# adrelino/mv-lm-icp

Hardware: AMD Instinct MI355X
Metric: ICP iterations/sec (NN+Jacobian+LM) (higher is better)
Workload: dtype f64; 1 GPU; cfg4: multiview 32 views x 200k pts, point-to-plane, SophusSE3 (E=62); views=32, pts_per_view=200000, edges=62, parallelism=single GPU, nn=auto

## Files before the change

mv-lm-icp_amd/csrc/api.cpp:

```cpp
#include <algorithm>
#include <cmath>
#include <cstring>
#include <ctime>
#include <chrono>
#include <condition_variable>
#include <exception>
#include <mutex>
#include <new>
#include <thread>

#include "common.h"
#include "comm.h"
#include "nn_tie.h"
#include "../host/se3.h"

namespace mvicp {

static thread_local char g_err[1024] = "";

void set_error(const char* fmt, ...) {
  va_list ap;
  va_start(ap, fmt);
  vsnprintf(g_err, sizeof(g_err), fmt, ap);
  va_end(ap);
}

int abi_exception() noexcept {
  try { throw; }
  catch (const std::bad_alloc&) { set_error("out of host memory"); }
  catch (const std::exception& e) { set_error("internal error: %s", e.what()); }
  catch (...) { set_error("internal error (unknown exception)"); }
  return MVICP_ERR_INTERNAL;
}

double search_bound(const mvicp_ctx* c, double d2_bound) {
  if (!(c->nn_search_factor > 0.0)) return 1.7976931348623157e308;
  const double f = std::max(1.0, c->nn_search_factor);
  const double b = d2_bound * f * f * (1.0 + 1e-9);
  return std::isfinite(b) ? b : 1.7976931348623157e308;
}

int cached_upload(mvicp_ctx* c, const char* key, const void* src, size_t bytes, void** dptr) {
  mvicp_ctx::CachedTable& t = c->tables[key];
  if (t.d && t.bytes.size() == bytes && std::memcmp(t.bytes.data(), src, bytes) == 0) { *dptr = t.d; return MVICP_OK; }
  MV_HIP(hipStreamSynchronize(c->stream));
  if (bytes > t.cap) {
    if (t.d) MV_HIP(hipFree(t.d));
    t.d = nullptr;
    MV_HIP(hipMalloc(&t.d, std::max<size_t>(bytes, 256)));
    t.cap = std::max<size_t>(bytes, 256);
  }
  MV_HIP(hipMemcpy(t.d, src, bytes, hipMemcpyHostToDevice));
  t.bytes.assign((const char*)src, (const char*)src + bytes);
  *dptr = t.d;
  return MVICP_OK;
}

void scratch_reset(mvicp_ctx* c) { c->scratch_used = 0; }

int scratch_upload(mvicp_ctx* c, const void* src, size_t bytes, void** dptr) {
  const size_t aligned = (bytes + 255) & ~(size_t)255;
  if (c->scratch_used + aligned > c->scratch_bytes) {
    if (c->scratch_used != 0) { set_error("scratch overflow (%zu + %zu > %zu)", c->scratch_used, aligned, c->scratch_bytes); return MVICP_ERR_STATE; }
    MV_HIP(hipStreamSynchronize(c->stream));
    if (c->d_scratch) MV_HIP(hipFree(c->d_scratch));
    c->scratch_bytes = std::max<size_t>(aligned * 4, 1 << 20);
    MV_HIP(hipMalloc((void**)&c->d_scratch, c->scratch_bytes));
  }
  void* d = c->d_scratch + c->scratch_used;
  MV_HIP(hipMemcpyAsync(d, src, bytes, hipMemcpyHostToDevice, c->stream));
  MV_HIP(hipStreamSynchronize(c->stream));
  c->scratch_used += aligned;
  *dptr = d;
  return MVICP_OK;
}

ProfScope::ProfScope(mvicp_ctx* ctx, const char* nm, double bytes) : c(ctx), name(nm), on(ctx->profile) {
  if (on && ctx->profile_level >= 2 && ((std::strncmp(nm, "nn_", 3) != 0 && std::strncmp(nm, "linearize", 9) != 0 && std::strcmp(nm, "comm") != 0) ||
                                        std::strcmp(nm, "nn_tie") == 0)) on = false;
  if (!on) return;
  ProfEntry& pe = c->prof[name];
  auto get = [&]() {
    hipEvent_t ev = nullptr;
    if (!pe.pool.empty()) { ev = pe.pool.back(); pe.pool.pop_back(); }
    else if (hipEventCreate(&ev) != hipSuccess) ev = nullptr;
    return ev;
  };
  a = get(); b = get();
  pe.bytes += bytes;
  if (std::strncmp(nm, "nn_", 3) == 0) { pe.survey_bytes += bytes; pe.queries += bytes / 36.0; }
  pe.launches += 1;
  if (a) (void)hipEventRecord(a, c->stream);
}
ProfScope::~ProfScope() {
  if (!on) return;
  if (b) (void)hipEventRecord(b, c->stream);
  if (a && b) c->prof[name].pending.push_back(std::make_pair(a, b));
}
static double now_ms() {
  timespec ts;
  clock_gettime(CLOCK_MONOTONIC, &ts);
  return ts.tv_sec * 1e3 + ts.tv_nsec * 1e-6;
}
HostScope::HostScope(mvicp_ctx* ctx, const char* nm) : c(ctx), name(nm), t0(0.0), on(ctx->profile) { if (on) t0 = now_ms(); }
HostScope::~HostScope() {
  if (!on) return;
  ProfEntry& pe = c->prof[name];
  pe.ms += now_ms() - t0;
  pe.launches += 1;
}
void prof_collect_lazy(mvicp_ctx* c) {
  for (auto& kv : c->prof) if (kv.second.pending.size() > 256) { prof_collect(c); return; }
}
void prof_collect(mvicp_ctx* c) {
  for (auto& kv : c->prof) {
    ProfEntry& pe = kv.second;
    for (auto& pr : pe.pending) {
      float ms = 0.f;
      if (hipEventSynchronize(pr.second) == hipSuccess && hipEventElapsedTime(&ms, pr.first, pr.second) == hipSuccess) pe.ms += ms;
      pe.pool.push_back(pr.first);
      pe.pool.push_back(pr.second);
    }
    pe.pending.clear();
  }
}

namespace {

template <typename T> int dev_alloc(T** p, size_t n) {
  *p = nullptr;
  if (n == 0) n = 1;
  MV_HIP(hipMalloc((void**)p, sizeof(T) * n));
  return MVICP_OK;
}
template <typename T> void dev_free(T*& p) {
  if (p) (void)hipFree(p);
  p = nullptr;
}

void free_graph(mvicp_ctx* c) {
  dev_free(c->d_esrc); dev_free(c->d_edst); dev_free(c->d_cap_off); dev_free(c->d_count);
  dev_free(c->d_ctl); c->d_nsrc = nullptr; c->d_a = nullptr; c->d_xf = nullptr; c->d_rel = nullptr; c->d_rel2 = nullptr; c->d_dirty = nullptr;
  dev_free(c->d_nn_idx); dev_free(c->d_nn_d2); dev_free(c->d_nn_lb); dev_free(c->d_first); dev_free(c->d_second);
  dev_free(c->d_sblock_off); dev_free(c->d_sel_keys1); dev_free(c->d_sel_keys2); c->n_sblocks = 0;
  dev_free(c->d_cd2); dev_free(c->d_qpos); dev_free(c->d_dirty_slots); dev_free(c->d_dslot_off); dev_free(c->d_stream); dev_free(c->d_cblock_off); dev_free(c->d_cblock_cnt); if (c->d_sel_state) (void)hipFree(c->d_sel_state);
  c->d_sel_state = nullptr; dev_free(c->d_sel_hist); dev_free(c->d_median); dev_free(c->d_chunk_edge); dev_free(c->d_chunk_start);
  dev_free(c->d_chunk_first); dev_free(c->d_partials); dev_free(c->d_out);
  if (c->h_pin) (void)hipHostFree(c->h_pin);
  c->h_pin = nullptr; c->h_pin_doubles = 0; c->d_res_host = nullptr; c->d_blocks_host = nullptr; c->lin_out = nullptr;
  c->census_pending = false; c->spec_ready = false; c->spec2_ready = false; c->spec_arm = false; c->d_spec_host = nullptr; c->d_adev_host = nullptr; c->d_res_target = nullptr; c->d_a_check = nullptr;
  dev_free(c->d_xblock_cnt); c->export_valid = false; c->export_in_flight = false; c->export_chunks = 0;
  for (hipEvent_t ev : c->export_events) (void)hipEventDestroy(ev);
  c->export_events.clear();
  if (c->d_export) (void)hipFree(c->d_export);
  if (c->h_export) (void)hipHostFree(c->h_export);
  c->d_export = nullptr; c->h_export = nullptr; c->export_cap = 0;
  c->E = 0; c->total_cap = 0; c->n_cblocks = 0; c->n_chunks = 0; c->have_corr = false;
}

int bind(mvicp_ctx* c) {
  if (!c) { set_error("null context"); return MVICP_ERR_ARG; }
  MV_HIP(hipSetDevice(c->device));
  return MVICP_OK;
}

double sqrt_bound(double t) {
  double x = t * t;
  while (std::sqrt(x) >= t && x > 0.0) x = std::nextafter(x, 0.0);
  while (std::sqrt(x) < t) x = std::nextafter(x, INFINITY);
  return x;
}

void inverse3(const double* m, double* r) {
#define M(i, j) m[(i) + 3 * (j)]
#define COF(i, j) (M(((i) + 1) % 3, ((j) + 1) % 3) * M(((i) + 2) % 3, ((j) + 2) % 3) - M(((i) + 1) % 3, ((j) + 2) % 3) * M(((i) + 2) % 3, ((j) + 1) % 3))
  const double c00 = COF(0, 0), c10 = COF(1, 0), c20 = COF(2, 0);
  const double det = (c00 * M(0, 0) + c10 * M(1, 0)) + c20 * M(2, 0);
  const double invdet = 1.0 / det;
  r[0] = c00 * invdet; r[3] = c10 * invdet; r[6] = c20 * invdet;
  r[1] = COF(0, 1) * invdet; r[4] = COF(1, 1) * invdet; r[7] = COF(2, 1) * invdet;
  r[2] = COF(0, 2) * invdet; r[5] = COF(1, 2) * invdet; r[8] = COF(2, 2) * invdet;
#undef COF
#undef M
}

void fill_query_xf(const double* Ps, const double* Pd, double* x) {
  double Rd[9];
  for (int j = 0; j < 3; ++j)
    for (int i = 0; i < 3; ++i) { x[i + 3 * j] = Ps[i + 4 * j]; Rd[i + 3 * j] = Pd[i + 4 * j]; }
  for (int i = 0; i < 3; ++i) { x[9 + i] = Ps[12 + i]; x[21 + i] = Pd[12 + i]; }
  inverse3(Rd, x + 12);
}

int ensure_pin(mvicp_ctx* c, size_t doubles) {
  if (doubles <= c->h_pin_doubles) return MVICP_OK;
  if (c->h_pin) MV_HIP(hipHostFree(c->h_pin));
  c->h_pin = nullptr;
  MV_HIP(hipHostMalloc((void**)&c->h_pin, sizeof(double) * doubles, hipHostMallocMapped));
  std::memset(c->h_pin, 0, sizeof(double) * doubles);
  c->h_pin_doubles = doubles;
  return MVICP_OK;
}

}

static void fill_rel_into(mvicp_ctx* c, const double* poses, double* h);
void fill_rel(mvicp_ctx* c, const double* poses) {
  fill_rel_into(c, poses, c->h_pin + c->ctl_r2_off);
}
static void fill_rel_into(mvicp_ctx* c, const double* poses, double* h) {
  for (int e = 0; e < c->E; ++e) {
    const double* Ps = poses + 16 * (size_t)c->esrc[e];
    const double* Pd = poses + 16 * (size_t)c->edst[e];
    double* r = h + (size_t)e * kEdgeRel;
    for (int j = 0; j < 3; ++j)
      for (int i = 0; i < 3; ++i) r[i + 3 * j] = Pd[0 + 4 * i] * Ps[0 + 4 * j] + Pd[1 + 4 * i] * Ps[1 + 4 * j] + Pd[2 + 4 * i] * Ps[2 + 4 * j];
    const double dt[3] = {Ps[12] - Pd[12], Ps[13] - Pd[13], Ps[14] - Pd[14]};
    for (int i = 0; i < 3; ++i) r[9 + i] = Pd[0 + 4 * i] * dt[0] + Pd[1 + 4 * i] * dt[1] + Pd[2 + 4 * i] * dt[2];
  }
}
int upload_rel(mvicp_ctx* c, const double* poses) {
  fill_rel(c, poses);
  MV_HIP(hipMemcpyAsync(c->d_rel, c->h_pin + c->ctl_r2_off, sizeof(double) * c->ctl_r2, hipMemcpyHostToDevice, c->stream));
  return MVICP_OK;
}

int stream_wait(mvicp_ctx* c) {
  if (c->spin_wait) {
    const double t0 = now_ms();
    for (;;) {
      const hipError_t q = hipStreamQuery(c->stream);
      if (q == hipSuccess) return MVICP_OK;
      if (q != hipErrorNotReady) { set_error("hipStreamQuery -> %s", hipGetErrorString(q)); return MVICP_ERR_HIP; }
      if (now_ms() - t0 > 2.0) break;
    }
  }
  MV_HIP(hipStreamSynchronize(c->stream));
  return MVICP_OK;
}

void census_resolve(mvicp_ctx* c) {
  if (!c->census_pending) return;
  c->census_pending = false;
  const unsigned long long* st = c->h_census;
  const double nq = c->census_nq;
  ProfEntry& pe = c->prof[c->census_scope];
  if (c->census_kind == 3) {
    const double hits = (double)st[3];
    pe.bytes += 36.0 * hits + 24.0 * (double)st[4] + 24.0 * (double)st[5] + 32.0 * (double)st[1];
    c->nn_candidates += (double)st[0]; c->nn_nodes += (double)st[1] + (double)st[5]; c->nn_far += (double)st[2]; c->nn_queries += nq; c->nn_hits += hits;
    c->nn_fetched += (double)st[4];
    pe.survey_bytes += 24.0 * (double)st[4] + 8.0 * ((double)st[1] + (double)st[5]);
  } else if (c->census_kind == 2) {
    c->nn_fetched += (double)st[0];
    pe.survey_bytes += 24.0 * (double)st[0] + 8.0 * (double)st[1];
    pe.bytes += 28.0 * (double)st[0] + 24.0 * (double)st[1];
    c->nn_candidates += (double)st[2]; c->nn_nodes += (double)st[1]; c->nn_queries += nq;
    for (int k = 0; k < 4; ++k) c->nn_dbg[k] += (double)st[4 + k];
    c->nn_hits += (double)st[3]; pe.bytes += 36.0 * (double)st[3];
  } else {
    const double hits = (double)st[3], searched = nq - hits;
    pe.bytes += 36.0 * hits + (c->census_kind == 1 ? 4.0 : 132.0) * searched + 32.0 * (double)st[0] + 32.0 * (double)st[1];
    c->nn_candidates += (double)st[0]; c->nn_nodes += (double)st[1]; c->nn_far += (double)st[2]; c->nn_queries += nq; c->nn_hits += hits;
    c->nn_fetched += (double)st[0];
    pe.survey_bytes += 24.0 * (double)st[0] + 8.0 * (double)st[1];
  }
}

namespace {
struct BuildSlots {
  std::mutex m; std::condition_variable cv; int free_slots;
  BuildSlots() : free_slots((int)std::max(2u, std::min(32u, std::thread::hardware_concurrency()))) {}
  void acquire() { std::unique_lock<std::mutex> lk(m); cv.wait(lk, [this]() { return free_slots > 0; }); --free_slots; }
  void release() { { std::lock_guard<std::mutex> lk(m); ++free_slots; } cv.notify_one(); }
};
BuildSlots& build_slots() { static BuildSlots s; return s; }
}

static int upload_sorted_normals(FrameDev& f, const double* nrm) {
  const int n = f.n;
  std::vector<double> sn(3 * (size_t)n);
  for (int i = 0; i < n; ++i) std::memcpy(&sn[3 * (size_t)i], nrm + 3 * (size_t)f.grid.h_order[i], 24);
  MV_HIP(hipMalloc((void**)&f.grid.snor, sizeof(double) * 3 * (size_t)std::max(n, 1)));
  MV_HIP(hipMemcpy(f.grid.snor, sn.data(), sizeof(double) * 3 * (size_t)n, hipMemcpyHostToDevice));
  return MVICP_OK;
}

static bool injected_build_failure(mvicp_ctx* c) {
  if (c->fault_inject_build.load() > 0 && c->fault_inject_build.fetch_sub(1) == 1) { set_error("injected structure-build failure (option fault_inject_build)"); return true; }
  return false;
}

static int build_frame_structures(mvicp_ctx* c, FrameDev& f, const double* xyz, const double* nrm) {
  if (injected_build_failure(c)) return MVICP_ERR_INTERNAL;
  const auto t0 = std::chrono::steady_clock::now();
  MV_CHECK(build_grid(c, f, xyz));
  if (nrm) MV_CHECK(upload_sorted_normals(f, nrm));
  f.build_ms[0] = std::chrono::duration<double, std::milli>(std::chrono::steady_clock::now() - t0).count();
  f.build_ms[1] = -1.0;
  return MVICP_OK;
}

static int build_frame_structures_device(mvicp_ctx* c, FrameDev& f, const DevBounds& b, int grid_curve, double grid_target) {
  if (injected_build_failure(c)) return MVICP_ERR_INTERNAL;
  return build_grid_device(c, f, b, grid_curve, grid_target);
}

int finish_builds(mvicp_ctx* c) {
  for (FrameDev& f : c->frames) {
    if (!f.job) continue;
    int s1 = MVICP_ERR_INTERNAL;
    try { s1 = f.job->fut.get(); } catch (...) { f.job->err = "structure build threw"; }
    if (s1 != MVICP_OK) {
      f.build_error = f.job->err.empty() ? std::string("structure build failed") : f.job->err;
      (void)hipSetDevice(c->device);
      free_grid(f.grid); f.has_grid = false;
    }
    f.job.reset();
  }
  for (size_t i = 0; i < c->frames.size(); ++i)
    if (!c->frames[i].build_error.empty()) {
      set_error("frame %d: %s (upload the cloud again with mvicp_set_frame)", (int)i, c->frames[i].build_error.c_str());
      return MVICP_ERR_STATE;
    }
  return MVICP_OK;
}

static void throttle_builds(mvicp_ctx* c) {
  const int limit = std::max(2, (int)std::min(32u, std::thread::hardware_concurrency()));
  for (;;) {
    int pending = 0;
    BuildJob* oldest = nullptr;
    for (FrameDev& f : c->frames)
      if (f.job && f.job->fut.valid() && f.job->fut.wait_for(std::chrono::seconds(0)) != std::future_status::ready) { if (!oldest) oldest = f.job.get(); ++pending; }
    if (pending < limit || !oldest) return;
    oldest->fut.wait();
  }
}

static int check_evaluable(mvicp_ctx* c, int plane) {
  if (!c->have_corr) { set_error("no correspondences: call mvicp_correspond or mvicp_set_correspondences first"); return MVICP_ERR_STATE; }
  if (plane) {
    for (int e = 0; e < c->E; ++e)
      if (c->owned[e] && c->h_count[e] > 0 && c->frames[c->edst[e]].grid.snor == nullptr) {
        set_error("point-to-plane needs normals on frame %d", c->edst[e]);
        return MVICP_ERR_STATE;
      }
  }
  return MVICP_OK;
}

int evaluate_pair(mvicp_ctx* c, const double* poses_a, const double* poses_b, int plane, int robust, double* out_a, double* out_b) {
  MV_CHECK(check_evaluable(c, plane));
  HostScope hs(c, "host.evaluate");
  const size_t n = (size_t)c->E * MVICP_EDGE_BLOCK;
  fill_rel_into(c, poses_b, c->h_pin + c->ctl_rel2_off);
  fill_rel(c, poses_a);
  MV_HIP(hipMemcpyAsync(c->d_rel2, c->h_pin + c->ctl_rel2_off, sizeof(double) * ((size_t)c->E * kEdgeRel + c->ctl_r2), hipMemcpyHostToDevice, c->stream));
  MV_CHECK(launch_linearize_pair(c, plane, robust, c->d_blocks_host, c->d_blocks2_host));
  MV_CHECK(stream_wait(c));
  std::memcpy(out_a, c->h_pin + c->pin_blocks_off, sizeof(double) * n);
  std::memcpy(out_b, c->h_pin + c->pin_blocks2_off, sizeof(double) * n);
  return MVICP_OK;
}

int evaluate_blocks(mvicp_ctx* c, const double* poses, int plane, int robust, double* out) {
  MV_CHECK(check_evaluable(c, plane));
  HostScope hs(c, "host.evaluate");
  const size_t n = (size_t)c->E * MVICP_EDGE_BLOCK;
  if (c->spec_ready) {
    c->spec_ready = false;
    if (plane == c->spec_q_plane && robust == c->spec_q_robust && c->spec_poses.size() == 16 * (size_t)c->n_frames &&
        std::memcmp(poses, c->spec_poses.data(), sizeof(double) * c->spec_poses.size()) == 0) {
      std::memcpy(out, c->h_pin + c->pin_spec_off, sizeof(double) * n);
      if (c->profile) c->prof["spec.hit"].launches += 1;
      return MVICP_OK;
    }
    c->spec2_ready = false;
  }
  if (c->spec2_ready) {
    c->spec2_ready = false;
    if (plane == c->spec2_plane && robust == c->spec2_robust && c->spec2_poses.size() == 16 * (size_t)c->n_frames &&
        std::memcmp(poses, c->spec2_poses.data(), sizeof(double) * c->spec2_poses.size()) == 0) {
      std::memcpy(out, c->h_pin + c->pin_spec2_off, sizeof(double) * n);
      if (c->profile) c->prof["spec2.hit"].launches += 1;
      c->last_cand_poses.assign(poses, poses + 16 * (size_t)c->n_frames); c->last_cand_plane = plane; c->last_cand_robust = robust;
      return MVICP_OK;
    }
  }
  c->last_cand_poses.assign(poses, poses + 16 * (size_t)c->n_frames); c->last_cand_plane = plane; c->last_cand_robust = robust;
  double* h = c->h_pin + c->pin_blocks_off;
  if (c->comm || c->ar_fn) {
    c->lin_out = c->d_out;
    int st_l = upload_rel(c, poses);
    if (st_l == MVICP_OK && c->fault_inject_eval > 0 && --c->fault_inject_eval == 0) { set_error("injected launch failure (option fault_inject_eval)"); st_l = MVICP_ERR_HIP; }
    if (st_l == MVICP_OK) st_l = launch_linearize(c, plane, robust);
    char local_msg[sizeof(g_err)] = "";
    if (st_l != MVICP_OK) std::memcpy(local_msg, g_err, sizeof(local_msg));
    if (hipMemsetAsync(c->d_out + n, st_l == MVICP_OK ? 0 : 0xFF, sizeof(double), c->stream) != hipSuccess) {
      if (st_l != MVICP_OK) return st_l;
      set_error("hipMemsetAsync of the poison slot failed"); return MVICP_ERR_HIP;
    }
    { ProfScope pc(c, "comm", 8.0 * (double)(n + 1)); MV_CHECK(comm_allreduce_sum(c, c->d_out, n + 1)); }
    double* hx = c->h_pin + c->pin_spec_off;
    MV_HIP(hipMemcpyAsync(hx, c->d_out, sizeof(double) * (n + 1), hipMemcpyDeviceToHost, c->stream));
    MV_CHECK(stream_wait(c));
    if (std::isnan(hx[n])) {
      if (st_l != MVICP_OK) { set_error("%s", local_msg); return st_l; }
      set_error("a peer rank failed before the exchange of this evaluation (poisoned exchange buffer)");
      return MVICP_ERR_COMM;
    }
    std::memcpy(out, hx, sizeof(double) * n);
    return MVICP_OK;
  } else {
    MV_CHECK(upload_rel(c, poses));
    c->lin_out = c->d_blocks_host;
    MV_CHECK(launch_linearize(c, plane, robust));
  }
  MV_CHECK(stream_wait(c));
  std::memcpy(out, h, sizeof(double) * n);
  return MVICP_OK;
}

}

using namespace mvicp;

extern "C" {

const char* mvicp_last_error(void) { return g_err; }
const char* mvicp_version(void) { return "mvicp_hip 0.5 (gfx950)"; }

int mvicp_create(int device, mvicp_ctx** out) try {
  if (!out) { set_error("out is null"); return MVICP_ERR_ARG; }
  *out = nullptr;
  int ndev = 0;
  hipError_t e = hipGetDeviceCount(&ndev);
  if (e != hipSuccess || ndev <= 0) {
    set_error("no HIP device available (%s): libmvicp_hip has no CPU fallback", e == hipSuccess ? "device count 0" : hipGetErrorString(e));
    return MVICP_ERR_HIP;
  }
  if (device < 0 || device >= ndev) { set_error("device %d out of range [0,%d)", device, ndev); return MVICP_ERR_ARG; }
  mvicp_ctx* c = new mvicp_ctx();
  c->device = device;
  MV_HIP(hipSetDevice(device));
  MV_HIP(hipStreamCreateWithFlags(&c->stream, hipStreamNonBlocking));
  *out = c;
  return MVICP_OK;
} MVICP_GUARD_ABI

int mvicp_destroy(mvicp_ctx* c) try {
  if (!c) return MVICP_OK;
  (void)hipSetDevice(c->device);
  (void)finish_builds(c);
  (void)hipStreamSynchronize(c->stream);
  comm_destroy(c);
  free_graph(c);
  for (FrameDev& f : c->frames) { dev_free(f.pts); dev_free(f.nor); free_grid(f.grid); free_tie(f); }
  dev_free(c->d_split_idx); dev_free(c->d_split_d2); dev_free(c->d_scratch);
  free_overlap(c);
  for (auto& kv : c->tables) if (kv.second.d) (void)hipFree(kv.second.d);
  if (c->d_census) (void)hipFree(c->d_census);
  if (c->h_census) (void)hipHostFree(c->h_census);
  if (c->d_tie_list) (void)hipFree(c->d_tie_list);
  if (c->d_tie_count) (void)hipFree(c->d_tie_count);
  if (c->h_tie_seen) (void)hipHostFree(c->h_tie_seen);
  if (c->h_far_seen) (void)hipHostFree(c->h_far_seen);
  if (c->d_far_list) (void)hipFree(c->d_far_list);
  if (c->d_far_count) (void)hipFree(c->d_far_count);
  for (auto& kv : c->prof) {
    for (auto& pr : kv.second.pending) { (void)hipEventDestroy(pr.first); (void)hipEventDestroy(pr.second); }
    for (hipEvent_t ev : kv.second.pool) (void)hipEventDestroy(ev);
  }
  (void)hipStreamDestroy(c->stream);
  delete c;
  return MVICP_OK;
} MVICP_GUARD_ABI

int mvicp_set_num_frames(mvicp_ctx* c, int n_frames) try {
  MV_CHECK(bind(c));
  if (n_frames < 0) { set_error("n_frames < 0"); return MVICP_ERR_ARG; }
  (void)finish_builds(c);
  if (c->E) free_graph(c);
  for (FrameDev& f : c->frames) { dev_free(f.pts); dev_free(f.nor); free_grid(f.grid); free_tie(f); }
  c->frames.assign(n_frames, FrameDev());
  c->n_frames = n_frames;
  return MVICP_OK;
} MVICP_GUARD_ABI

int mvicp_set_frame(mvicp_ctx* c, int frame, const double* xyz, const double* nrm, int n) try {
  MV_CHECK(bind(c));
  if (frame < 0 || frame >= c->n_frames) { set_error("frame %d out of range [0,%d)", frame, c->n_frames); return MVICP_ERR_ARG; }
  if (n < 0 || (n > 0 && !xyz)) { set_error("bad cloud (n=%d)", n); return MVICP_ERR_ARG; }
  if (c->E) { set_error("set frames before mvicp_set_graph"); return MVICP_ERR_STATE; }
  FrameDev& f = c->frames[frame];
  if (f.job) { try { (void)f.job->fut.get(); } catch (...) {} f.job.reset(); }
  dev_free(f.pts); dev_free(f.nor); free_grid(f.grid); free_tie(f);
  f.has_grid = false; f.build_error.clear();
  f.n = n;
  MV_CHECK(dev_alloc(&f.pts, 3 * (size_t)n));
  if (n) MV_HIP(hipMemcpy(f.pts, xyz, sizeof(double) * 3 * (size_t)n, hipMemcpyHostToDevice));
  if (nrm) {
    MV_CHECK(dev_alloc(&f.nor, 3 * (size_t)n));
    if (n) MV_HIP(hipMemcpy(f.nor, nrm, sizeof(double) * 3 * (size_t)n, hipMemcpyHostToDevice));
  }
  f.max_norm = 0.0;
  for (int i = 0; i < n; ++i) {
    const double* p = xyz + 3 * (size_t)i;
    if (!std::isfinite(p[0]) || !std::isfinite(p[1]) || !std::isfinite(p[2])) { set_error("non-finite coordinate in cloud"); return MVICP_ERR_ARG; }
    f.max_norm = std::max(f.max_norm, std::sqrt(p[0] * p[0] + p[1] * p[1] + p[2] * p[2]));
  }
  if (n == 0) return MVICP_OK;
  if (!c->async_build) {
    const int st = build_frame_structures(c, f, xyz, nrm);
    if (st != MVICP_OK) { f.build_error = g_err; free_grid(f.grid); f.has_grid = false; }
    return st;
  }
  throttle_builds(c);
  std::shared_ptr<BuildJob> job = std::make_shared<BuildJob>();
  job->xyz.assign(xyz, xyz + 3 * (size_t)n);
  if (nrm) job->nrm.assign(nrm, nrm + 3 * (size_t)n);
  FrameDev* fp = &f;
  BuildJob* jp = job.get();
  job->fut = std::async(std::launch::async, [c, fp, jp]() -> int {
    build_slots().acquire();
    int st = MVICP_ERR_INTERNAL;
    try {
      st = hipSetDevice(c->device) == hipSuccess ? build_frame_structures(c, *fp, jp->xyz.data(), jp->nrm.empty() ? nullptr : jp->nrm.data()) : MVICP_ERR_HIP;
      if (st != MVICP_OK) jp->err = g_err;
    } catch (const std::exception& e) { jp->err = std::string("structure build: ") + e.what(); }
    catch (...) { jp->err = "structure build threw"; }
    std::vector<double>().swap(jp->xyz); std::vector<double>().swap(jp->nrm);
    build_slots().release();
    return st;
  });
  f.job = job;
  return MVICP_OK;
} MVICP_GUARD_ABI

static int check_device_pointer(mvicp_ctx* c, const void* p, const char* what) {
  hipPointerAttribute_t at;
  std::memset(&at, 0, sizeof(at));
  const hipError_t e = hipPointerGetAttributes(&at, p);
  if (e != hipSuccess) {
    (void)hipGetLastError();
    set_error("%s is not a device pointer (%s)", what, hipGetErrorString(e));
    return MVICP_ERR_ARG;
  }
  if (at.type != hipMemoryTypeDevice) { set_error("%s is not device memory (memory type %d)", what, (int)at.type); return MVICP_ERR_ARG; }
  if (at.device != c->device) { set_error("%s lives on device %d, the context on device %d", what, at.device, c->device); return MVICP_ERR_ARG; }
  return MVICP_OK;
}

int mvicp_set_frame_device(mvicp_ctx* c, int frame, const double* d_xyz, const double* d_nrm, int n) try {
  MV_CHECK(bind(c));
  if (frame < 0 || frame >= c->n_frames) { set_error("frame %d out of range [0,%d)", frame, c->n_frames); return MVICP_ERR_ARG; }
  if (n < 0 || (n > 0 && !d_xyz)) { set_error("bad cloud (n=%d)", n); return MVICP_ERR_ARG; }
  if (c->E) { set_error("set frames before mvicp_set_graph"); return MVICP_ERR_STATE; }
  if (n > 0) {
    MV_CHECK(check_device_pointer(c, d_xyz, "xyz"));
    if (d_nrm) MV_CHECK(check_device_pointer(c, d_nrm, "nrm"));
  }
  FrameDev& f = c->frames[frame];
  if (f.job) { try { (void)f.job->fut.get(); } catch (...) {} f.job.reset(); }
  dev_free(f.pts); dev_free(f.nor); free_grid(f.grid); free_tie(f);
  f.has_grid = false; f.build_error.clear();
  f.n = n;
  f.max_norm = 0.0;
  MV_CHECK(dev_alloc(&f.pts, 3 * (size_t)n));
  if (n) MV_HIP(hipMemcpyAsync(f.pts, d_xyz, sizeof(double) * 3 * (size_t)n, hipMemcpyDeviceToDevice, c->stream));
  if (d_nrm) {
    MV_CHECK(dev_alloc(&f.nor, 3 * (size_t)n));
    if (n) MV_HIP(hipMemcpyAsync(f.nor, d_nrm, sizeof(double) * 3 * (size_t)n, hipMemcpyDeviceToDevice, c->stream));
  }
  if (n == 0) { MV_HIP(hipStreamSynchronize(c->stream)); return MVICP_OK; }
  const auto t0 = std::chrono::steady_clock::now();
  DevBounds b;
  MV_CHECK(device_bounds(c->stream, f.pts, n, &b));
  b.wall_ms = std::chrono::duration<double, std::milli>(std::chrono::steady_clock::now() - t0).count();
  if (b.nonfinite) { set_error("non-finite coordinate in cloud"); return MVICP_ERR_ARG; }
  f.max_norm = b.max_norm;
  const int curve = c->grid_curve;
  const double target = c->grid_target;
  if (!c->async_build) {
    const int st = build_frame_structures_device(c, f, b, curve, target);
    if (st != MVICP_OK) { f.build_error = g_err; free_grid(f.grid); f.has_grid = false; }
    return st;
  }
  throttle_builds(c);
  std::shared_ptr<BuildJob> job = std::make_shared<BuildJob>();
  FrameDev* fp = &f;
  BuildJob* jp = job.get();
  job->fut = std::async(std::launch::async, [c, fp, jp, b, curve, target]() -> int {
    build_slots().acquire();
    int st = MVICP_ERR_INTERNAL;
    try {
      st = hipSetDevice(c->device) == hipSuccess ? build_frame_structures_device(c, *fp, b, curve, target) : MVICP_ERR_HIP;
      if (st != MVICP_OK) jp->err = g_err;
    } catch (const std::exception& e) { jp->err = std::string("structure build: ") + e.what(); }
    catch (...) { jp->err = "structure build threw"; }
    build_slots().release();
    return st;
  });
  f.job = job;
  return MVICP_OK;
} MVICP_GUARD_ABI

long long mvicp_get_structure(mvicp_ctx* c, int frame, const char* name, void* out, long long cap_bytes) try {
  MV_CHECK(bind(c));
  if (frame < 0 || frame >= c->n_frames || !name) { set_error("frame %d out of range [0,%d) or no name", frame, c->n_frames); return MVICP_ERR_ARG; }
  MV_CHECK(finish_builds(c));
  const FrameDev& f = c->frames[frame];
  if (!f.has_grid) { set_error("frame %d has no structures (n = %d)", frame, f.n); return MVICP_ERR_STATE; }
  const GridDev& G = f.grid;
  const size_t n = (size_t)f.n;
  const void* dsrc = nullptr; const void* hsrc = nullptr; size_t bytes = 0;
  std::vector<double> sc;
  const int tiles = (f.n + 31) / 32, blocks = (tiles + 63) / 64;
  if (!std::strcmp(name, "spts")) { dsrc = G.spts; bytes = 24 * n; }
  else if (!std::strcmp(name, "sidx")) { dsrc = G.sidx; bytes = 4 * n; }
  else if (!std::strcmp(name, "srec")) { dsrc = G.srec; bytes = sizeof(PointRec) * n; }
  else if (!std::strcmp(name, "crec")) { dsrc = G.crec; bytes = sizeof(PointRec) * n; }
  else if (!std::strcmp(name, "inv")) { dsrc = G.inv; bytes = 4 * n; }
  else if (!std::strcmp(name, "snor")) { dsrc = G.snor; bytes = G.snor ? 24 * n : 0; }
  else if (!std::strcmp(name, "table")) { dsrc = G.table; bytes = 16 * ((size_t)G.table_mask + 1); }
  else if (!std::strcmp(name, "oct")) { dsrc = G.oct; bytes = 32 * (size_t)(8 * G.oct_first_leaf + 1); }
  else if (!std::strcmp(name, "wide")) { dsrc = G.wide; bytes = 4 * (size_t)(G.wide_off[G.wide_levels - 1] + 6ll * G.wide_cnt[G.wide_levels - 1]); }
  else if (!std::strcmp(name, "mf_ops")) { dsrc = G.mf_ops; bytes = (size_t)std::max(tiles, 1) * 64 * 16; }
  else if (!std::strcmp(name, "mf_blk")) { dsrc = G.mf_blk; bytes = (size_t)std::max(blocks, 1) * 48; }
  else if (!std::strcmp(name, "bricks")) { dsrc = G.bricks; bytes = G.bricks ? 16 * (size_t)G.bdims[0] * G.bdims[1] * G.bdims[2] : 0; }
  else if (!std::strcmp(name, "celltab")) { dsrc = G.celltab; bytes = G.celltab ? G.celltab_bytes : 0; }
  else if (!std::strcmp(name, "h_order")) { hsrc = G.h_order.data(); bytes = 4 * G.h_order.size(); }
  else if (!std::strcmp(name, "h_inv")) { hsrc = G.h_inv.data(); bytes = 4 * G.h_inv.size(); }
  else if (!std::strcmp(name, "scalars") || !std::strcmp(name, "build_ms")) {
    if (name[0] == 's') {
      for (int a = 0; a < 3; ++a) sc.push_back(G.dims[a]);
      for (int a = 0; a < 3; ++a) sc.push_back(G.origin[a]);
      sc.push_back(G.cell); sc.push_back(G.inv_cell); sc.push_back(G.n_cells); sc.push_back(G.table_mask); sc.push_back(G.table_shift);
      sc.push_back(G.oct_leaf); sc.push_back((double)G.oct_first_leaf); sc.push_back(G.wide_levels);
      for (int l = 0; l < 6; ++l) sc.push_back(G.wide_cnt[l]);
      for (int l = 0; l < 6; ++l) sc.push_back((double)G.wide_off[l]);
      sc.push_back(G.maxabs); sc.push_back(G.struct_bytes); sc.push_back(f.max_norm);
      for (int a = 0; a < 3; ++a) sc.push_back(G.bdims[a]);
    } else {
      sc.push_back(f.build_ms[0]); sc.push_back(f.build_ms[1]);
    }
    hsrc = sc.data(); bytes = sizeof(double) * sc.size();
  } else { set_error("unknown structure name \"%s\"", name); return MVICP_ERR_ARG; }
  if (!out) return (long long)bytes;
  if (cap_bytes < (long long)bytes) { set_error("%s: %zu bytes do not fit in %lld", name, bytes, cap_bytes); return MVICP_ERR_ARG; }
  if (bytes == 0) return 0;
  if (hsrc) std::memcpy(out, hsrc, bytes);
  else {
    MV_HIP(hipStreamSynchronize(c->stream));
    MV_HIP(hipMemcpy(out, dsrc, bytes, hipMemcpyDeviceToHost));
  }
  return (long long)bytes;
} MVICP_GUARD_ABI

int mvicp_recompute_normals(mvicp_ctx* c, int frame, int k, double* nrm_out, int* knn_out) try {
  MV_CHECK(bind(c));
  if (frame < 0 || frame >= c->n_frames) { set_error("frame %d out of range", frame); return MVICP_ERR_ARG; }
  MV_CHECK(finish_builds(c));
  FrameDev& f = c->frames[frame];
  if (f.n < k) { set_error("frame %d has %d points < k = %d (common.h:333 asserts >= 3)", frame, f.n, k); return MVICP_ERR_STATE; }
  if (!f.nor) MV_CHECK(dev_alloc(&f.nor, 3 * (size_t)f.n));
  if (!f.grid.snor) MV_CHECK(dev_alloc(&f.grid.snor, 3 * (size_t)f.n));
  int* d_knn = nullptr;
  if (knn_out) MV_CHECK(dev_alloc(&d_knn, (size_t)f.n * k));
  int st = launch_normals(c, f, k, d_knn);
  if (st == MVICP_OK) {
    hipError_t e = hipStreamSynchronize(c->stream);
    if (e == hipSuccess && nrm_out) e = hipMemcpy(nrm_out, f.nor, sizeof(double) * 3 * (size_t)f.n, hipMemcpyDeviceToHost);
    if (e == hipSuccess && knn_out) e = hipMemcpy(knn_out, d_knn, sizeof(int) * (size_t)f.n * k, hipMemcpyDeviceToHost);
    if (e != hipSuccess) { set_error("recompute_normals: %s", hipGetErrorString(e)); st = MVICP_ERR_HIP; }
  }
  dev_free(d_knn);
  c->spec_ready = false; c->spec2_ready = false;
  if (st == MVICP_OK && c->E > 0) {
    bool any = false;
    std::vector<int> dirty(c->E, 0);
    for (int e = 0; e < c->E; ++e)
      if (c->owned[e] && c->edst[e] == frame) { c->list_valid[e] = 0; if (c->have_corr && c->h_count[e] > 0) { dirty[e] = 1; any = true; } }
    if (any) {
      MV_HIP(hipMemcpy(c->d_dirty, dirty.data(), sizeof(int) * c->E, hipMemcpyHostToDevice));
      MV_CHECK(launch_gather_stream(c));
      MV_HIP(hipStreamSynchronize(c->stream));
    }
  }
  if (c->profile) prof_collect_lazy(c);
  return st;
} MVICP_GUARD_ABI

int mvicp_set_shard(mvicp_ctx* c, int rank, int world) try {
  MV_CHECK(bind(c));
  if (world < 1 || rank < 0 || rank >= world) { set_error("bad shard %d/%d", rank, world); return MVICP_ERR_ARG; }
  if (c->E) { set_error("call mvicp_set_shard before mvicp_set_graph"); return MVICP_ERR_STATE; }
  c->rank = rank; c->world = world;
  return MVICP_OK;
} MVICP_GUARD_ABI

int mvicp_edge_owner(int n_edges, const int* n_src, int world, int* owner) try {
  if (n_edges < 0 || world < 1 || (n_edges > 0 && (!n_src || !owner))) { set_error("bad arguments"); return MVICP_ERR_ARG; }
  double total = 0, cum = 0;
  for (int e = 0; e < n_edges; ++e) total += n_src[e];
  for (int e = 0; e < n_edges; ++e) {
    const double n = n_src[e];
    int o = total > 0 ? (int)std::floor((cum + 0.5 * n) * world / total) : 0;
    owner[e] = std::min(std::max(o, 0), world - 1);
    cum += n;
  }
  return MVICP_OK;
} MVICP_GUARD_ABI

int mvicp_overlap(mvicp_ctx* c, const double* poses, float thresh, int max_samples, int* samples, int* hits, long long* sumq, int* q_exp) try {
  MV_CHECK(bind(c));
  if (!poses || !samples || !hits) { set_error("poses / samples / hits is null"); return MVICP_ERR_ARG; }
  if (!std::isfinite(thresh) || !(thresh > 0.f)) { set_error("thresh must be finite and > 0"); return MVICP_ERR_ARG; }
  const int K = c->n_frames;
  if (K <= 0) { set_error("no frames: call mvicp_set_num_frames first"); return MVICP_ERR_STATE; }
  for (size_t k = 0; k < 16 * (size_t)K; ++k)
    if (!std::isfinite(poses[k])) { set_error("non-finite pose entry (frame %d)", (int)(k / 16)); return MVICP_ERR_ARG; }
  for (int i = 0; i < K; ++i)
    if (!c->frames[i].pts) { set_error("frame %d was never uploaded", i); return MVICP_ERR_STATE; }
  MV_CHECK(finish_builds(c));
  const double B2 = sqrt_bound((double)thresh);
  int ex = 0;
  (void)std::frexp(B2, &ex);
  const int q = 31 - ex;
  if (q_exp) *q_exp = q;
  std::vector<double> xf(24 * (size_t)K * K, 0.0);
  for (int i = 0; i < K; ++i)
    for (int j = 0; j < K; ++j)
      if (i != j) fill_query_xf(poses + 16 * (size_t)i, poses + 16 * (size_t)j, &xf[24 * ((size_t)i * K + j)]);
  return overlap_census(c, xf.data(), B2, std::ldexp(1.0, q), max_samples, samples, hits, sumq);
} MVICP_GUARD_ABI

int mvicp_graph_from_overlap(int n_frames, const int* samples, const int* hits, const long long* sumq, int knn, double min_fraction,
                             int skip_frame0, int cap, int* src, int* dst, int* n_components) try {
  const int K = n_frames;
  if (K < 0 || knn < 0 || cap < 0 || (K > 0 && (!samples || !hits)) || !(min_fraction == min_fraction)) { set_error("bad arguments"); return MVICP_ERR_ARG; }
  std::vector<int> parent((size_t)K);
  for (int i = 0; i < K; ++i) parent[i] = i;
  auto root = [&](int a) { while (parent[a] != a) { parent[a] = parent[parent[a]]; a = parent[a]; } return a; };
  int n_edges = 0;
  std::vector<int> cand;
  for (int i = 0; i < K; ++i) {
    cand.clear();
    const int* h = hits + (size_t)i * K;
    const long long* sq = sumq ? sumq + (size_t)i * K : nullptr;
    for (int j = 0; j < K; ++j)
      if (j != i && h[j] > 0 && (double)h[j] >= min_fraction * (double)samples[i]) cand.push_back(j);
    std::sort(cand.begin(), cand.end(), [&](int a, int b) {
      if (h[a] != h[b]) return h[a] > h[b];
      if (sq && sq[a] != sq[b]) return sq[a] < sq[b];
      return a < b;
    });
    const int take = std::min<int>(knn, (int)cand.size());
    for (int k = 0; k < take; ++k) {
      parent[root(i)] = root(cand[k]);
      if (i == 0 && skip_frame0) continue;
      if (n_edges >= cap) { set_error("more than cap = %d edges (frame %d of %d, knn = %d)", cap, i, K, knn); return MVICP_ERR_ARG; }
      if (!src || !dst) { set_error("src / dst is null"); return MVICP_ERR_ARG; }
      src[n_edges] = i; dst[n_edges] = cand[k]; ++n_edges;
    }
  }
  if (n_components) {
    int comps = 0;
    for (int i = 0; i < K; ++i) comps += root(i) == i ? 1 : 0;
    *n_components = comps;
  }
  return n_edges;
} MVICP_GUARD_ABI

int mvicp_set_graph(mvicp_ctx* c, int n_edges, const int* src, const int* dst) try {
  MV_CHECK(bind(c));
  if (n_edges < 0 || (n_edges > 0 && (!src || !dst))) { set_error("bad edge list"); return MVICP_ERR_ARG; }
  for (int e = 0; e < n_edges; ++e)
    if (src[e] < 0 || src[e] >= c->n_frames || dst[e] < 0 || dst[e] >= c->n_frames || src[e] == dst[e]) {
      set_error("edge %d (%d->%d) invalid", e, src[e], dst[e]);
      return MVICP_ERR_ARG;
    }
  MV_CHECK(finish_builds(c));
  free_graph(c);
  const int E = n_edges;
  c->E = E;
  c->esrc.assign(src, src + E);
  c->edst.assign(dst, dst + E);
  c->owned.assign(E, 0);
  c->active.assign(E, 0);
  c->h_count.assign(E, 0);
  c->h_weight.assign(E, 0.f);
  {
    std::vector<int> ns(E), owner(E);
    for (int e = 0; e < E; ++e) ns[e] = c->frames[src[e]].n;
    MV_CHECK(mvicp_edge_owner(E, ns.data(), c->world, owner.data()));
    for (int e = 0; e < E; ++e) c->owned[e] = owner[e] == c->rank;
  }
  {
    double total = 0;
    for (int e = 0; e < E; ++e) total += c->frames[src[e]].n;
    c->lin_chunk = total >= 6e6 ? 8192 : total >= 2e6 ? 4096 : total >= 5e5 ? 1024 : 512;
    if (c->lin_chunk_override > 0) c->lin_chunk = c->lin_chunk_override;
  }
  const int kLinChunk = c->lin_chunk;
  c->cap_off.assign(E + 1, 0);
  c->cblock_off.assign(E + 1, 0);
  c->chunk_first.assign(E + 1, 0);
  std::vector<int> chunk_edge, chunk_start;
  for (int e = 0; e < E; ++e) {
    const long long n = c->owned[e] ? c->frames[src[e]].n : 0;
    c->cap_off[e + 1] = c->cap_off[e] + ((n + 63) / 64) * 64;
    c->cblock_off[e + 1] = c->cblock_off[e] + (int)((n + kCompactBlock - 1) / kCompactBlock);
    const int nch = (int)((n + kLinChunk - 1) / kLinChunk);
    c->chunk_first[e + 1] = c->chunk_first[e] + nch;
    for (int k = 0; k < nch; ++k) { chunk_edge.push_back(e); chunk_start.push_back(k * kLinChunk); }
  }
  c->total_cap = c->cap_off[E];
  c->n_cblocks = c->cblock_off[E];
  c->n_chunks = c->chunk_first[E];
  if (c->lin_interleave) {
    std::vector<int> ce, cs;
    for (int e0 = 0; e0 < E;) {
      int e1 = e0 + 1;
      while (e1 < E && src[e1] == src[e0]) ++e1;
      int maxc = 0;
      for (int e = e0; e < e1; ++e) maxc = std::max(maxc, c->chunk_first[e + 1] - c->chunk_first[e]);
      for (int g = 0; g < maxc; g += 8)
        for (int e = e0; e < e1; ++e) {
          const int nch = c->chunk_first[e + 1] - c->chunk_first[e];
          for (int k = g; k < std::min(g + 8, nch); ++k) { ce.push_back(e); cs.push_back(k * kLinChunk); }
        }
      e0 = e1;
    }
    chunk_edge.swap(ce); chunk_start.swap(cs);
  }
  const size_t cap = (size_t)c->total_cap;
  MV_CHECK(dev_alloc(&c->d_esrc, E)); MV_CHECK(dev_alloc(&c->d_edst, E)); MV_CHECK(dev_alloc(&c->d_cap_off, E + 1));
  MV_CHECK(dev_alloc(&c->d_count, E));
  c->ctl_r1 = (size_t)E * kEdgeXf + (size_t)E + 2 * (size_t)E;
  c->ctl_rel2_off = (c->ctl_r1 + 1) & ~(size_t)1;
  c->ctl_r2_off = c->ctl_rel2_off + (size_t)E * kEdgeRel;
  c->ctl_r2 = (size_t)E * (kEdgeRel + 1);
  MV_CHECK(dev_alloc(&c->d_ctl, c->ctl_r2_off + c->ctl_r2));
  MV_HIP(hipMemset(c->d_ctl, 0, sizeof(double) * std::max<size_t>(c->ctl_r2_off + c->ctl_r2, 1)));
  c->d_xf = c->d_ctl; c->d_nsrc = reinterpret_cast<int*>(c->d_ctl + (size_t)E * kEdgeXf); c->d_dirty = c->d_nsrc + E;
  c->d_sel_lohi = c->d_ctl + (size_t)E * (kEdgeXf + 1);
  c->sel_med1.assign(E, -1.0); c->sel_med2.assign(E, -1.0);
  c->d_rel = c->d_ctl + c->ctl_r2_off; c->d_a = c->d_rel + (size_t)E * kEdgeRel; c->d_rel2 = c->d_ctl + c->ctl_rel2_off;
  MV_CHECK(dev_alloc(&c->d_nn_idx, cap)); MV_CHECK(dev_alloc(&c->d_nn_d2, cap)); MV_CHECK(dev_alloc(&c->d_nn_lb, cap));
  c->nn_cache_valid = false; c->prev_q.assign((size_t)E * 12, 0.0); c->nn_cache_edge.assign(E, 0);
  c->auto_prev_dist = 0.0; c->auto_last_method = -1; c->corr_tie_seen = c->corr_far_seen = 1u;
  MV_CHECK(dev_alloc(&c->d_first, cap)); MV_CHECK(dev_alloc(&c->d_second, cap)); MV_CHECK(dev_alloc(&c->d_cd2, cap));
  MV_CHECK(dev_alloc(&c->d_stream, 10 * cap));
  MV_CHECK(dev_alloc(&c->d_qpos, cap));
  MV_HIP(hipMemset(c->d_qpos, 0xff, sizeof(int) * std::max<size_t>(cap, 1)));
  c->list_valid.assign(E, 0); c->explicit_list.assign(E, 0); c->export_valid = false; c->export_off.assign((size_t)E + 1, 0);
  c->qpos_valid.assign(E, 0); c->corr_epoch.assign(E, 0);
  for (int e = 0; e < E; ++e) c->corr_epoch[e] = ++c->epoch_counter;
  c->dslot_off.assign(E + 1, 0);
  for (int e = 0; e < E; ++e) c->dslot_off[e + 1] = c->dslot_off[e] + (int)(((c->owned[e] ? c->frames[src[e]].n : 0) + 255) / 256);
  c->n_dslots = c->dslot_off[E];
  MV_CHECK(dev_alloc(&c->d_dirty_slots, (size_t)c->n_dslots)); MV_CHECK(dev_alloc(&c->d_dslot_off, (size_t)E + 1));
  MV_HIP(hipMemset(c->d_dirty_slots, 0, sizeof(int) * std::max<size_t>((size_t)c->n_dslots, 1)));
  MV_HIP(hipMemcpy(c->d_dslot_off, c->dslot_off.data(), sizeof(int) * (E + 1), hipMemcpyHostToDevice));
  MV_CHECK(dev_alloc(&c->d_cblock_off, E + 1)); MV_CHECK(dev_alloc(&c->d_cblock_cnt, (size_t)c->n_cblocks));
  MV_HIP(hipMalloc(&c->d_sel_state, 16 * 3 * (size_t)std::max(E, 1))); MV_CHECK(dev_alloc(&c->d_sel_hist, (size_t)E * (3 * 2048 + 5)));
  c->sblock_off.assign(E + 1, 0);
  for (int e = 0; e < E; ++e) c->sblock_off[e + 1] = c->sblock_off[e] + (int)(((c->owned[e] ? c->frames[src[e]].n : 0) + kSelBlock - 1) / kSelBlock);
  c->n_sblocks = c->sblock_off[E];
  MV_CHECK(dev_alloc(&c->d_sblock_off, (size_t)E + 1));
  MV_HIP(hipMemcpy(c->d_sblock_off, c->sblock_off.data(), sizeof(int) * (E + 1), hipMemcpyHostToDevice));
  MV_CHECK(dev_alloc(&c->d_sel_keys1, cap)); MV_CHECK(dev_alloc(&c->d_sel_keys2, cap));
  if (cap > c->far_cap) {
    if (c->d_far_list) MV_HIP(hipFree(c->d_far_list));
    c->d_far_list = nullptr; c->far_cap = 0;
    MV_HIP(hipMalloc(&c->d_far_list, sizeof(int) * 2 * cap));
    c->far_cap = cap;
  }
  MV_CHECK(warm_nn_grid(c)); MV_CHECK(warm_nn_tile(c)); MV_CHECK(warm_nn_mfma(c));
  if (c->tie_rule && !(c->tie_lazy && c->world == 1)) {
    std::vector<int> need;
    for (int e = 0; e < E; ++e) if (c->owned[e]) need.push_back(dst[e]);
    MV_CHECK(ensure_tie_trees(c, need));
  }
  MV_CHECK(dev_alloc(&c->d_median, E));
  MV_CHECK(dev_alloc(&c->d_chunk_edge, (size_t)c->n_chunks)); MV_CHECK(dev_alloc(&c->d_chunk_start, (size_t)c->n_chunks));
  MV_CHECK(dev_alloc(&c->d_chunk_first, E + 1));
  MV_CHECK(dev_alloc(&c->d_partials, 2 * (size_t)c->n_chunks * kLinPartial));
  MV_CHECK(dev_alloc(&c->d_out, (size_t)E * (MVICP_EDGE_BLOCK + 3) + 2));
  MV_HIP(hipMemset(c->d_out, 0, sizeof(double) * ((size_t)E * (MVICP_EDGE_BLOCK + 3) + 2)));
  if (E) {
    MV_HIP(hipMemcpy(c->d_esrc, src, sizeof(int) * E, hipMemcpyHostToDevice));
    MV_HIP(hipMemcpy(c->d_edst, dst, sizeof(int) * E, hipMemcpyHostToDevice));
    MV_HIP(hipMemset(c->d_count, 0, sizeof(int) * E));
  }
  MV_HIP(hipMemcpy(c->d_cap_off, c->cap_off.data(), sizeof(long long) * (E + 1), hipMemcpyHostToDevice));
  MV_HIP(hipMemcpy(c->d_cblock_off, c->cblock_off.data(), sizeof(int) * (E + 1), hipMemcpyHostToDevice));
  MV_HIP(hipMemcpy(c->d_chunk_first, c->chunk_first.data(), sizeof(int) * (E + 1), hipMemcpyHostToDevice));
  if (c->n_chunks) {
    MV_HIP(hipMemcpy(c->d_chunk_edge, chunk_edge.data(), sizeof(int) * c->n_chunks, hipMemcpyHostToDevice));
    MV_HIP(hipMemcpy(c->d_chunk_start, chunk_start.data(), sizeof(int) * c->n_chunks, hipMemcpyHostToDevice));
  }
  c->pin_blocks_off = c->ctl_r2_off + c->ctl_r2;
  c->pin_res_off = c->pin_blocks_off + (size_t)E * MVICP_EDGE_BLOCK;
  c->pin_misc_off = c->pin_res_off + 2 * (size_t)E + 2;
  c->pin_spec_off = c->pin_misc_off + 4 * (size_t)E + 64;
  c->pin_adev_off = c->pin_spec_off + (size_t)E * (MVICP_EDGE_BLOCK + 3) + 2;
  if (c->h_pin) { MV_HIP(hipHostFree(c->h_pin)); c->h_pin = nullptr; c->h_pin_doubles = 0; }
  c->pin_spec2_off = (c->pin_adev_off + (size_t)E + 8 + 1) & ~(size_t)1;
  c->pin_rel2_off = c->pin_spec2_off + (size_t)E * MVICP_EDGE_BLOCK + ((size_t)E * MVICP_EDGE_BLOCK & 1);
  c->pin_blocks2_off = (c->pin_rel2_off + (size_t)E * kEdgeRel + 1) & ~(size_t)1;
  MV_CHECK(ensure_pin(c, c->pin_blocks2_off + (size_t)E * MVICP_EDGE_BLOCK + 8));
  {
    void* dp = nullptr;
    MV_HIP(hipHostGetDevicePointer(&dp, c->h_pin, 0));
    c->d_blocks_host = (double*)dp + c->pin_blocks_off;
    c->d_res_host = (double*)dp + c->pin_res_off;
    c->d_spec_host = (double*)dp + c->pin_spec_off;
    c->d_adev_host = (double*)dp + c->pin_adev_off;
    c->d_spec2_host = (double*)dp + c->pin_spec2_off;
    c->d_blocks2_host = (double*)dp + c->pin_blocks2_off;
  }
  c->spec_ready = false; c->spec_arm = false; c->bracket_counters_clean = false;
  c->spec2_ready = false; c->spec2_armed = false; c->last_cand_poses.clear();
  c->prev_xf.assign((size_t)E * 24, 0.0);
  if (!c->h_census) MV_HIP(hipHostMalloc((void**)&c->h_census, 8 * sizeof(unsigned long long), hipHostMallocDefault));
  return MVICP_OK;
} MVICP_GUARD_ABI

static void forget_history(mvicp_ctx* c) {
  const int E = c->E;
  c->nn_cache_valid = false; c->nn_cache_thresh = -1.f;
  c->prev_q.assign((size_t)E * 12, 0.0); c->prev_xf.assign((size_t)E * 24, 0.0);
  c->nn_cache_edge.assign(E, 0);
  c->auto_prev_dist = 0.0; c->auto_last_method = -1; c->last_rms = -1.0; c->prev_grid_kernel = false;
  c->corr_tie_seen = c->corr_far_seen = 1u;
  c->list_valid.assign(E, 0);
  c->export_valid = false;
  c->qpos_valid.assign(E, 0);
  for (int e = 0; e < E; ++e) c->corr_epoch[e] = ++c->epoch_counter;
  c->sel_med1.assign(E, -1.0); c->sel_med2.assign(E, -1.0);
  c->spec_ready = false; c->spec_arm = false; c->spec_flags_valid = false;
  c->spec2_ready = false; c->spec2_armed = false; c->last_cand_poses.clear();
  c->have_corr = false;
  std::fill(c->h_count.begin(), c->h_count.end(), 0); std::fill(c->h_weight.begin(), c->h_weight.end(), 0.f);
}

int mvicp_reset_history(mvicp_ctx* c) try {
  MV_CHECK(bind(c));
  MV_HIP(hipStreamSynchronize(c->stream));
  forget_history(c);
  return MVICP_OK;
} MVICP_GUARD_ABI

static int correspond_once(mvicp_ctx* c, const double* poses, const unsigned char* fixed, float thresh, int nn_method, int* counts, float* weights, bool* tie_unresolved);

int mvicp_correspond(mvicp_ctx* c, const double* poses, const unsigned char* fixed, float thresh, int nn_method, int* counts, float* weights) try {
  MV_CHECK(bind(c));
  bool unresolved = false;
  MV_CHECK(correspond_once(c, poses, fixed, thresh, nn_method, counts, weights, &unresolved));
  if (!unresolved) return MVICP_OK;
  std::vector<int> need;
  for (int e = 0; e < c->E; ++e) if (c->active[e] && !c->frames[c->edst[e]].has_tie) need.push_back(c->edst[e]);
  MV_HIP(hipStreamSynchronize(c->stream));
  MV_CHECK(ensure_tie_trees(c, need));
  forget_history(c);
  unresolved = false;
  MV_CHECK(correspond_once(c, poses, fixed, thresh, nn_method, counts, weights, &unresolved));
  if (unresolved) { set_error("tie fix-up still without a tree after building them"); return MVICP_ERR_INTERNAL; }
  return MVICP_OK;
} MVICP_GUARD_ABI

static int correspond_once(mvicp_ctx* c, const double* poses, const unsigned char* fixed, float thresh, int nn_method, int* counts, float* weights, bool* tie_unresolved) {
  if (!poses) { set_error("poses is null"); return MVICP_ERR_ARG; }
  if (c->E == 0) { set_error("no graph: call mvicp_set_graph first"); return MVICP_ERR_STATE; }
  const int E = c->E;
  HostScope hs_all(c, "host.correspond");
  std::vector<int> nsrc(E, 0);
  std::vector<char> same_edge(E, 0);
  std::vector<char> unchanged(E, 0);
  const bool hist_ok = c->have_corr && (int)c->nn_cache_edge.size() == E && c->nn_cache_thresh == thresh && (int)c->qpos_valid.size() == E;
  std::vector<double> eps_ratio;
  bool same_active_set = (int)c->nn_cache_edge.size() == E;
  double* hx = c->h_pin;
  for (int e = 0; e < E; ++e) {
    c->active[e] = c->owned[e] && !(fixed && fixed[c->esrc[e]]);
    if (same_active_set && (c->active[e] != 0) != (c->nn_cache_edge[e] != 0)) same_active_set = false;
    nsrc[e] = c->active[e] ? c->frames[c->esrc[e]].n : 0;
    const double* Ps = poses + 16 * (size_t)c->esrc[e];
    const double* Pd = poses + 16 * (size_t)c->edst[e];
    double* x = hx + (size_t)e * kEdgeXf;
    fill_query_xf(Ps, Pd, x);
    double Mq[12];
    for (int j = 0; j < 3; ++j)
      for (int i = 0; i < 3; ++i) Mq[i + 3 * j] = x[12 + i] * x[0 + 3 * j] + x[12 + i + 3] * x[1 + 3 * j] + x[12 + i + 6] * x[2 + 3 * j];
    const double dt[3] = {x[9] - x[21], x[10] - x[22], x[11] - x[23]};
    for (int i = 0; i < 3; ++i) Mq[9 + i] = x[12 + i] * dt[0] + x[12 + i + 3] * dt[1] + x[12 + i + 6] * dt[2];
    double* pq = &c->prev_q[(size_t)e * 12];
    double scale = 0.0;
    for (int k = 0; k < 12; ++k) { x[25 + k] = Mq[k] - pq[k]; scale = std::max(scale, std::fabs(Mq[k])); }
    const double rmax = c->frames[c->esrc[e]].max_norm;
    if (c->active[e]) {
      double fro = 0.0;
      for (int k = 0; k < 9; ++k) fro += x[25 + k] * x[25 + k];
      const double eps_e = std::sqrt(fro) * rmax + std::sqrt(x[34] * x[34] + x[35] * x[35] + x[36] * x[36]);
      const double mu_e = c->tile_mu * c->frames[c->edst[e]].grid.cell;
      eps_ratio.push_back(mu_e > 0.0 ? eps_e / mu_e : 1e300);
    }
    const bool cache_on = c->nn_cache_valid && c->nn_cache_enable && c->active[e] && (int)c->nn_cache_edge.size() == E && c->nn_cache_edge[e] &&
                          c->nn_cache_thresh == thresh;
    double* pxf = &c->prev_xf[(size_t)e * 24];
    if (!c->owned[e]) unchanged[e] = 1;
    else if (c->active[e]) unchanged[e] = hist_ok && c->nn_cache_edge[e] && c->qpos_valid[e] && !c->explicit_list[e] && std::memcmp(pxf, x, sizeof(double) * 24) == 0;
    else unchanged[e] = hist_ok && !c->nn_cache_edge[e] && !c->explicit_list[e] && c->h_count[e] == 0;
    const bool same_xf = cache_on && std::memcmp(pxf, x, sizeof(double) * 24) == 0;
    x[24] = cache_on ? (same_xf ? 0.0 : 1e-12 * (scale * (rmax + 1.0) + 1.0)) : -1.0;
    same_edge[e] = same_xf;
    std::memcpy(pxf, x, sizeof(double) * 24);
    for (int k = 37; k < kEdgeXf; ++k) x[k] = 0.0;
    std::memcpy(pq, Mq, sizeof(Mq));
  }
  int* hn = reinterpret_cast<int*>(hx + (size_t)E * kEdgeXf);
  int* hd = hn + E;
  std::memcpy(hn, nsrc.data(), sizeof(int) * E);

  int st_local = MVICP_OK;
  if (c->tie_rule && !(c->tie_lazy && c->world == 1)) {
    std::vector<int> need;
    for (int e = 0; e < E; ++e) if (c->active[e] && !c->frames[c->edst[e]].has_tie) need.push_back(c->edst[e]);
    if (!need.empty()) st_local = ensure_tie_trees(c, need);
  }
  const double bound = sqrt_bound((double)thresh);
  double t_mark = now_ms();
  auto mark = [&](const char* nm) { if (c->profile) { const double t = now_ms(); ProfEntry& pe = c->prof[nm]; pe.ms += t - t_mark; pe.launches += 1; t_mark = t; } };
  mark("host.corr.setup");
  int method = nn_method;
  if (method == MVICP_NN_AUTO) {
    method = MVICP_NN_TILE;
    if (c->have_corr) {
      double dist = 0.0, cell = 0.0;
      int m = 0;
      for (int e = 0; e < E; ++e)
        if (c->h_count[e] > 0) { dist += c->h_weight[e] / 1.5; cell += c->frames[c->edst[e]].grid.cell; ++m; }
      if (m > 0) {
        dist /= m; cell /= m;
        const bool settled = c->auto_prev_dist > 0.0 ? dist > c->auto_settle * c->auto_prev_dist : dist < 0.5 * cell;
        if (c->nn_cell) {
          double pred = dist;
          if (c->last_rms >= 0.0) pred = std::min(pred, std::sqrt(c->last_rms * c->last_rms + 0.09 * cell * cell));
          if (pred < c->auto_switch * cell || c->auto_last_method == MVICP_NN_GRID) method = MVICP_NN_GRID;
        } else if (dist < 1.5 * cell && (settled || c->auto_last_method == MVICP_NN_GRID)) method = MVICP_NN_GRID;
        c->auto_prev_dist = dist;
      }
    }
  }
  if (method == MVICP_NN_GRID || method == MVICP_NN_TILE) {
    for (int e = 0; e < E; ++e)
      if (c->active[e] && (!c->frames[c->edst[e]].has_grid || !c->frames[c->esrc[e]].has_grid)) method = MVICP_NN_BRUTE;
  }
  bool tile_lb = false, handed_over = false;
  if (nn_method == MVICP_NN_AUTO && method == MVICP_NN_GRID && c->auto_last_method == MVICP_NN_TILE && c->tile_bounds >= 1 &&
      c->nn_cache_enable && !c->nn_cell) { method = MVICP_NN_TILE; tile_lb = true; handed_over = true; }
  if (method == MVICP_NN_TILE && c->tile_bounds >= 2 && c->nn_cache_enable) tile_lb = true;
  bool tile_cached = false;
  bool all_same = true;
  {
    for (int e = 0; e < E; ++e) if (c->active[e] && !same_edge[e]) all_same = false;
    if (nn_method == MVICP_NN_AUTO && method == MVICP_NN_GRID && !handed_over && c->tile_cache && c->tile_bounds >= 1 && c->nn_cache_valid &&
        c->nn_cache_enable && !c->nn_cell && !all_same) { method = MVICP_NN_TILE; tile_lb = true; tile_cached = true; handed_over = true; }
    if (method == MVICP_NN_TILE && !tile_cached && c->tile_cache >= 2 && tile_lb && c->nn_cache_valid && c->nn_cache_enable && !all_same) tile_cached = true;
  }
  {
    std::vector<int> dirty(E, 1);
    if ((method == MVICP_NN_TILE || (method == MVICP_NN_GRID && !c->nn_tree_only && !c->nn_skip_far)) && c->list_reuse)
      for (int e = 0; e < E; ++e) if (c->active[e] && c->list_valid[e]) dirty[e] = 0;
    std::memcpy(hd, dirty.data(), sizeof(int) * E);
  }
  bool use_bracket = c->sel_bracket && c->have_corr;
  {
    double* lohi = hx + (size_t)E * (kEdgeXf + 1);
    for (int e = 0; e < E; ++e) {
      lohi[2 * e] = lohi[2 * e + 1] = 0.0;
      if (!c->active[e]) continue;
      const double m1 = c->sel_med1[e], m2 = c->sel_med2[e];
      if (!(m1 > 0.0 && m2 > 0.0 && std::fabs(m1 - m2) <= 0.001 * m1)) { use_bracket = false; continue; }
      lohi[2 * e] = m1 * 0.994; lohi[2 * e + 1] = m1 * 1.006;
    }
  }
  bool nothing_can_change = method == MVICP_NN_GRID && c->list_reuse && !c->nn_tree_only && !c->nn_skip_far && same_active_set && !c->nn_cell;
  for (int e = 0; e < E && nothing_can_change; ++e)
    if (c->active[e] && !(same_edge[e] && hd[e] == 0)) nothing_can_change = false;
  c->skip_dirty_reduce = nothing_can_change;
  c->tie_skip = nothing_can_change && c->corr_tie_seen == 0u;
  c->far_skip = nothing_can_change && c->corr_far_seen == 0u && c->prev_grid_kernel && method == MVICP_NN_GRID;
  const bool tie_launched = c->tie_rule && !c->tie_skip, far_launched = method == MVICP_NN_GRID && !c->far_skip;
  const bool exchange = c->comm != nullptr || c->ar_fn != nullptr;
  c->spec_ready = false; c->spec2_ready = false;
  c->spec_arm = c->spec_enable && c->spec_flags_valid;
  if (c->spec_arm && c->spec_plane)
    for (int e = 0; e < E; ++e) if (!(fixed && fixed[c->esrc[e]]) && c->frames[c->edst[e]].n > 0 && c->frames[c->edst[e]].grid.snor == nullptr) c->spec_arm = false;
  const size_t nb = (size_t)E * MVICP_EDGE_BLOCK, ntail = 3 * (size_t)E + 1;
  c->d_res_target = exchange ? c->d_out + nb : nullptr;
  c->d_a_check = exchange ? c->d_out + nb + 2 * (size_t)E + 1 : c->d_adev_host;
  size_t upload_doubles = c->ctl_r1;
  bool spec2_plan = false;
  if (c->spec_arm) {
    c->spec_poses.resize(16 * (size_t)c->n_frames);
    double xp[7];
    for (int k = 0; k < c->n_frames; ++k) { se3::pose_to_x(c->spec_param, poses + 16 * (size_t)k, xp); se3::x_to_pose(c->spec_param, xp, &c->spec_poses[16 * (size_t)k]); }
    fill_rel(c, c->spec_poses.data());
    c->spec_q_plane = c->spec_plane; c->spec_q_robust = c->spec_robust;
    upload_doubles = c->ctl_r2_off + (size_t)E * kEdgeRel;
    spec2_plan = !exchange && c->spec2_enable && all_same && same_active_set && c->have_corr && c->last_cand_poses.size() == 16 * (size_t)c->n_frames &&
                 c->last_cand_plane == c->spec_q_plane && c->last_cand_robust == c->spec_q_robust;
    if (spec2_plan && c->lin_pair) fill_rel_into(c, c->last_cand_poses.data(), hx + c->ctl_rel2_off);
  }
  if (method != MVICP_NN_BRUTE && method != MVICP_NN_GRID && method != MVICP_NN_TILE) { set_error("unknown nn_method %d", nn_method); return MVICP_ERR_ARG; }
  bool all_unchanged = true;
  for (int e = 0; e < E; ++e) { if (!unchanged[e]) all_unchanged = false; if (c->active[e]) c->qpos_valid[e] = 0; }
  auto local_search = [&]() -> int {
  MV_HIP(hipMemcpyAsync(c->d_ctl, hx, sizeof(double) * upload_doubles, hipMemcpyHostToDevice, c->stream));
  c->far_narrow = nn_method == MVICP_NN_AUTO && method == MVICP_NN_GRID && c->nn_cache_valid && c->nn_cache_enable && all_same;
  if (c->fault_inject > 0 && --c->fault_inject == 0) { set_error("injected launch failure (option fault_inject)"); return MVICP_ERR_HIP; }
  if (method == MVICP_NN_BRUTE) MV_CHECK(launch_nn_brute_edges(c));
  else if (method == MVICP_NN_GRID) MV_CHECK(launch_nn_grid_edges(c, bound));
  else {
    c->cached_on_mfma = false;
    if (tile_cached && c->tile_mfma == 1 && c->cache_mfma_ratio > 0.0 && !eps_ratio.empty()) {
      std::nth_element(eps_ratio.begin(), eps_ratio.begin() + eps_ratio.size() / 2, eps_ratio.end());
      const double med = eps_ratio[eps_ratio.size() / 2];
      if (c->profile) { ProfEntry& pe = c->prof["auto.eps_over_mu"]; pe.ms = med; pe.launches += 1; }
      c->cached_on_mfma = med > c->cache_mfma_ratio;
    }
    MV_CHECK(launch_nn_tile_edges(c, bound, tile_lb, tile_cached, c->list_reuse));
  }
  c->tie_skip = false; c->far_skip = false;
  c->prev_grid_kernel = method == MVICP_NN_GRID;
  c->last_rms = -1.0;
  c->nn_cache_valid = ((method == MVICP_NN_GRID) && !c->nn_tree_only && !c->nn_skip_far) || tile_lb;
  c->nn_cache_thresh = thresh;
  c->auto_last_method = handed_over ? MVICP_NN_GRID : method;
  c->nn_cache_edge.assign(c->active.begin(), c->active.end());
  for (int e = 0; e < E; ++e) { c->list_valid[e] = c->active[e]; if (c->owned[e]) c->qpos_valid[e] = c->active[e]; if (c->active[e]) c->explicit_list[e] = 0; }
  if (!all_unchanged) c->export_valid = false;

  mark("host.corr.nn_launch");
  if (!nothing_can_change) {
    MV_CHECK(launch_compact(c, bound));
    MV_CHECK(launch_gather_stream(c));
  }
  return use_bracket ? launch_select_bracket(c) : launch_select_median(c);
  };
  if (st_local == MVICP_OK) st_local = local_search();
  if (st_local != MVICP_OK && !exchange) { c->spec_flags_valid = false; return st_local; }
  int st_q = MVICP_OK;
  char local_msg[sizeof(g_err)] = "";
  if (exchange) {
    c->lin_out = c->d_out;
    if (st_local == MVICP_OK) {
      if (c->spec_arm) st_local = launch_linearize(c, c->spec_q_plane, c->spec_q_robust);
      else {
        if (hipMemsetAsync(c->d_out, 0, sizeof(double) * nb, c->stream) != hipSuccess ||
            hipMemsetAsync(c->d_out + nb + 2 * (size_t)E + 1, 0, sizeof(double) * (size_t)E, c->stream) != hipSuccess) { set_error("hipMemsetAsync of the exchange buffer failed"); st_local = MVICP_ERR_HIP; }
      }
    }
    if (st_local != MVICP_OK) {
      std::memcpy(local_msg, g_err, sizeof(local_msg));
      if (hipMemsetAsync(c->d_out + nb + 2 * (size_t)E, 0xFF, sizeof(double), c->stream) != hipSuccess) {
        set_error("%s — and the exchange buffer could not be poisoned: the peers of this rank will block in the collective", local_msg);
        c->spec_flags_valid = false; c->spec_arm = false;
        return st_local;
      }
    }
    { ProfScope pc(c, "comm", 8.0 * (double)(nb + ntail)); st_q = comm_allreduce_sum(c, c->d_out, nb + ntail); }
    if (st_q == MVICP_OK && hipMemcpyAsync(c->h_pin + c->pin_spec_off, c->d_out, sizeof(double) * (nb + ntail), hipMemcpyDeviceToHost, c->stream) != hipSuccess) {
      set_error("hipMemcpyAsync of the exchanged buffer failed"); st_q = MVICP_ERR_HIP;
    }
  } else if (c->spec_arm && spec2_plan && c->lin_pair) {
    c->spec2_armed = false;
    st_q = launch_linearize_pair(c, c->spec_q_plane, c->spec_q_robust, c->d_spec_host, c->d_spec2_host);
    if (st_q == MVICP_OK) { c->spec2_armed = true; c->spec2_poses = c->last_cand_poses; c->spec2_plane = c->spec_q_plane; c->spec2_robust = c->spec_q_robust; }
  } else if (c->spec_arm) {
    c->lin_out = c->d_spec_host;
    st_q = launch_linearize(c, c->spec_q_plane, c->spec_q_robust);
    c->spec2_armed = false;
    if (st_q == MVICP_OK && spec2_plan) {
      fill_rel_into(c, c->last_cand_poses.data(), c->h_pin + c->pin_rel2_off);
      if (hipMemcpyAsync(c->d_rel, c->h_pin + c->pin_rel2_off, sizeof(double) * (size_t)E * kEdgeRel, hipMemcpyHostToDevice, c->stream) == hipSuccess) {
        c->lin_out = c->d_spec2_host;
        st_q = launch_linearize(c, c->spec_q_plane, c->spec_q_robust);
        if (st_q == MVICP_OK) { c->spec2_armed = true; c->spec2_poses = c->last_cand_poses; c->spec2_plane = c->spec_q_plane; c->spec2_robust = c->spec_q_robust; }
      }
    }
  }
  mark("host.corr.post_launch");
  if (st_q == MVICP_OK) st_q = stream_wait(c);
  if (st_q != MVICP_OK) { c->spec_flags_valid = false; c->spec_arm = false; return st_q; }
  if (exchange && std::isnan(c->h_pin[c->pin_spec_off + nb + 2 * (size_t)E])) {
    forget_history(c);
    c->census_pending = false;
    if (st_local != MVICP_OK) { set_error("%s", local_msg); return st_local; }
    set_error("a peer rank failed before the exchange of this search (poisoned exchange buffer); nothing was updated, cross-round state dropped on every rank");
    return MVICP_ERR_COMM;
  }
  census_resolve(c);
  if (tie_launched) c->corr_tie_seen = c->h_tie_seen ? *c->h_tie_seen : 1u;
  if (tie_launched && c->h_tie_seen && c->h_tie_seen[1] != 0u) *tie_unresolved = true;
  if (far_launched) c->corr_far_seen = c->h_far_seen ? *c->h_far_seen : 1u;
  else if (method != MVICP_NN_GRID) c->corr_far_seen = 1u;
  mark("host.corr.wait");
  const double* hr = exchange ? c->h_pin + c->pin_spec_off + nb : c->h_pin + c->pin_res_off;
  bool spec_bad = false;
  {
    bool redo = false;
    for (int e = 0; e < E; ++e) if (hr[2 * e + 1] < 0.0) redo = true;
    if (redo) {
      spec_bad = true;
      int st_r = launch_select_median(c);
      if (exchange) {
        int st_x = MVICP_OK;
        if (st_r != MVICP_OK) {
          std::memcpy(local_msg, g_err, sizeof(local_msg));
          if (hipMemsetAsync(c->d_out + nb + 2 * (size_t)E, 0xFF, sizeof(double), c->stream) != hipSuccess) { c->spec_flags_valid = false; c->spec_arm = false; return st_r; }
        }
        { ProfScope pc(c, "comm", 8.0 * (double)ntail); st_x = comm_allreduce_sum(c, c->d_out + nb, ntail); }
        if (st_x == MVICP_OK && hipMemcpyAsync(c->h_pin + c->pin_spec_off + nb, c->d_out + nb, sizeof(double) * ntail, hipMemcpyDeviceToHost, c->stream) != hipSuccess) {
          set_error("hipMemcpyAsync of the exchanged tail failed"); st_x = MVICP_ERR_HIP;
        }
        if (st_x == MVICP_OK) st_x = stream_wait(c);
        if (st_x != MVICP_OK) { c->spec_flags_valid = false; c->spec_arm = false; return st_x; }
        if (std::isnan(hr[2 * (size_t)E])) {
          forget_history(c);
          if (st_r != MVICP_OK) { set_error("%s", local_msg); return st_r; }
          set_error("a peer rank failed before the second exchange of this search (poisoned exchange buffer); cross-round state dropped on every rank");
          return MVICP_ERR_COMM;
        }
      } else {
        if (st_r == MVICP_OK) st_r = stream_wait(c);
        if (st_r != MVICP_OK) { c->spec_flags_valid = false; c->spec_arm = false; return st_r; }
      }
    }
  }
  for (int e = 0; e < E; ++e) {
    if (!(c->owned[e] && c->active[e])) { c->sel_med1[e] = c->sel_med2[e] = -1.0; continue; }
    c->sel_med2[e] = c->sel_med1[e];
    c->sel_med1[e] = hr[2 * e] > 0 ? hr[2 * e + 1] : -1.0;
  }
  std::vector<double> pack(2 * (size_t)E, 0.0);
  for (int e = 0; e < E; ++e)
    if (exchange || (c->owned[e] && c->active[e])) { pack[2 * e] = hr[2 * e]; pack[2 * e + 1] = hr[2 * e] > 0 ? hr[2 * e + 1] : 0.0; }
  if (c->spec_arm) {
    const double* ad = exchange ? hr + 2 * (size_t)E + 1 : c->h_pin + c->pin_adev_off;
    if (hr[2 * (size_t)E] != (double)(exchange ? c->world : 1)) spec_bad = true;
    for (int e = 0; e < E && !spec_bad; ++e)
      if (exchange || (c->owned[e] && c->active[e])) {
        const double a_host = pack[2 * e] > 0 ? (double)(float)(std::sqrt(pack[2 * e + 1]) * 1.5) : 0.0;
        if (ad[e] != a_host) spec_bad = true;
      }
  }
  c->spec_ready = c->spec_arm && !spec_bad;
  c->spec2_ready = c->spec_ready && c->spec2_armed;
  c->spec2_armed = false;
  c->spec_arm = false;
  double* ha = c->h_pin + c->ctl_r2_off + (size_t)E * kEdgeRel;
  for (int e = 0; e < E; ++e) {
    c->h_count[e] = (int)pack[2 * e];
    const double nth = std::sqrt(pack[2 * e + 1]);
    c->h_weight[e] = c->h_count[e] > 0 ? (float)(nth * 1.5) : 0.f;
    ha[e] = (double)c->h_weight[e];
    if (counts) counts[e] = c->h_count[e];
    if (weights) weights[e] = c->h_weight[e];
  }
  for (int e = 0; e < E; ++e) if (!unchanged[e]) c->corr_epoch[e] = ++c->epoch_counter;
  c->have_corr = true;
  mark("host.corr.finish");
  if (c->profile) prof_collect_lazy(c);
  return MVICP_OK;
}

static int ensure_export(mvicp_ctx* c, bool wait = true) {
  if (!c->export_valid) {
    HostScope hs(c, "host.export");
    MV_CHECK(launch_export(c));
    c->export_valid = true;
  }
  if (wait && c->export_in_flight) {
    MV_CHECK(stream_wait(c));
    c->export_in_flight = false;
    if (c->profile) prof_collect_lazy(c);
  }
  return MVICP_OK;
}

int mvicp_map_correspondences(mvicp_ctx* c, const mvicp_corr** triples, const long long** offsets) try {
  MV_CHECK(bind(c));
  if (!triples || !offsets) { set_error("null output"); return MVICP_ERR_ARG; }
  if (!c->have_corr) { set_error("no correspondences yet"); return MVICP_ERR_STATE; }
  MV_CHECK(ensure_export(c));
  *triples = (const mvicp_corr*)c->h_export;
  *offsets = c->export_off.data();
  return MVICP_OK;
} MVICP_GUARD_ABI

int mvicp_map_correspondences_async(mvicp_ctx* c, const mvicp_corr** triples, const long long** offsets) try {
  MV_CHECK(bind(c));
  if (!triples || !offsets) { set_error("null output"); return MVICP_ERR_ARG; }
  if (!c->have_corr) { set_error("no correspondences yet"); return MVICP_ERR_STATE; }
  MV_CHECK(ensure_export(c, false));
  *triples = (const mvicp_corr*)c->h_export;
  *offsets = c->export_off.data();
  return MVICP_OK;
} MVICP_GUARD_ABI

int mvicp_wait_correspondences(mvicp_ctx* c, int edge) try {
  MV_CHECK(bind(c));
  if (edge < 0 || edge >= c->E) { set_error("edge %d out of range", edge); return MVICP_ERR_ARG; }
  if (!c->export_valid) { set_error("no export in flight: call mvicp_map_correspondences_async after the search"); return MVICP_ERR_STATE; }
  if (!c->export_in_flight || c->export_chunks == 0) return MVICP_OK;
  const int k = c->export_edge_chunk[edge];
  MV_HIP(hipEventSynchronize(c->export_events[k]));
  if (k == c->export_chunks - 1) c->export_in_flight = false;
  return MVICP_OK;
} MVICP_GUARD_ABI

int mvicp_correspondence_epochs(mvicp_ctx* c, const unsigned long long** epochs) try {
  MV_CHECK(bind(c));
  if (!epochs) { set_error("null output"); return MVICP_ERR_ARG; }
  if (c->E == 0) { set_error("no graph"); return MVICP_ERR_STATE; }
  *epochs = c->corr_epoch.data();
  return MVICP_OK;
} MVICP_GUARD_ABI

int mvicp_get_correspondences(mvicp_ctx* c, int edge, int cap, int* first, int* second, double* dist) try {
  MV_CHECK(bind(c));
  if (edge < 0 || edge >= c->E) { set_error("edge %d out of range", edge); return MVICP_ERR_ARG; }
  if (!c->have_corr) { set_error("no correspondences yet"); return MVICP_ERR_STATE; }
  if (!c->owned[edge]) { set_error("edge %d is owned by another rank", edge); return MVICP_ERR_STATE; }
  const int n = c->h_count[edge];
  if (cap < n) { set_error("capacity %d < count %d", cap, n); return MVICP_ERR_ARG; }
  if (!c->explicit_list[edge]) {
    if (n == 0) return 0;
    MV_CHECK(ensure_export(c));
    const mvicp_corr* t = (const mvicp_corr*)c->h_export + c->export_off[edge];
    if (c->export_off[edge + 1] - c->export_off[edge] != n) { set_error("export of edge %d holds %lld triples, expected %d", edge, c->export_off[edge + 1] - c->export_off[edge], n); return MVICP_ERR_STATE; }
    for (int i = 0; i < n; ++i) {
      if (first) first[i] = t[i].first;
      if (second) second[i] = t[i].second;
      if (dist) dist[i] = t[i].dist;
    }
    return n;
  }
  const size_t off = (size_t)c->cap_off[edge];
  MV_HIP(hipStreamSynchronize(c->stream));
  std::vector<int> a(n), b(n);
  std::vector<double> d(n);
  if (n) {
    MV_HIP(hipMemcpy(a.data(), c->d_first + off, sizeof(int) * n, hipMemcpyDeviceToHost));
    MV_HIP(hipMemcpy(b.data(), c->d_second + off, sizeof(int) * n, hipMemcpyDeviceToHost));
    MV_HIP(hipMemcpy(d.data(), c->d_cd2 + off, sizeof(double) * n, hipMemcpyDeviceToHost));
  }
  const std::vector<int>& so = c->frames[c->esrc[edge]].grid.h_order;
  const std::vector<int>& dorder = c->frames[c->edst[edge]].grid.h_order;
  std::vector<int> perm(n);
  for (int i = 0; i < n; ++i) { a[i] = so[a[i]]; b[i] = dorder[b[i]]; perm[i] = i; }
  std::stable_sort(perm.begin(), perm.end(), [&](int x, int y) { return a[x] < a[y]; });
  for (int i = 0; i < n; ++i) {
    const int k = perm[i];
    if (first) first[i] = a[k];
    if (second) second[i] = b[k];
    if (dist) dist[i] = std::sqrt(d[k]);
  }
  return n;
} MVICP_GUARD_ABI

int mvicp_set_correspondences(mvicp_ctx* c, int edge, int n, const int* first, const int* second, float weight) try {
  MV_CHECK(bind(c));
  if (edge < 0 || edge >= c->E) { set_error("edge %d out of range", edge); return MVICP_ERR_ARG; }
  if (!c->owned[edge]) { set_error("edge %d is owned by another rank", edge); return MVICP_ERR_STATE; }
  const int ns = c->frames[c->esrc[edge]].n, nd = c->frames[c->edst[edge]].n;
  if (n < 0 || n > ns) { set_error("n=%d exceeds the edge capacity N_src=%d", n, ns); return MVICP_ERR_ARG; }
  for (int i = 0; i < n; ++i)
    if (first[i] < 0 || first[i] >= ns || second[i] < 0 || second[i] >= nd) { set_error("correspondence %d out of range", i); return MVICP_ERR_ARG; }
  const size_t off = (size_t)c->cap_off[edge];
  MV_HIP(hipStreamSynchronize(c->stream));
  if (n) {
    const std::vector<int>& si = c->frames[c->esrc[edge]].grid.h_inv;
    const std::vector<int>& di = c->frames[c->edst[edge]].grid.h_inv;
    std::vector<int> a(n), b(n);
    for (int i = 0; i < n; ++i) { a[i] = si[first[i]]; b[i] = di[second[i]]; }
    MV_HIP(hipMemcpy(c->d_first + off, a.data(), sizeof(int) * n, hipMemcpyHostToDevice));
    MV_HIP(hipMemcpy(c->d_second + off, b.data(), sizeof(int) * n, hipMemcpyHostToDevice));
    MV_HIP(hipMemset(c->d_cd2 + off, 0, sizeof(double) * n));
  }
  c->nn_cache_valid = false;
  c->spec_ready = false; c->spec2_ready = false;
  c->list_valid[edge] = 0; c->explicit_list[edge] = 1; c->export_valid = false;
  c->qpos_valid[edge] = 0; c->corr_epoch[edge] = ++c->epoch_counter;
  c->sel_med1[edge] = c->sel_med2[edge] = -1.0;
  const double a = (double)weight;
  MV_HIP(hipMemcpy(c->d_count + edge, &n, sizeof(int), hipMemcpyHostToDevice));
  {
    const int not_identity = -1;
    MV_HIP(hipMemcpy(c->d_nsrc + edge, &not_identity, sizeof(int), hipMemcpyHostToDevice));
  }
  MV_HIP(hipMemcpy(c->d_a + edge, &a, sizeof(double), hipMemcpyHostToDevice));
  c->h_pin[c->ctl_r2_off + (size_t)c->E * kEdgeRel + edge] = a;
  c->h_count[edge] = n;
  c->h_weight[edge] = weight;
  c->have_corr = true;
  const int one = 1;
  MV_HIP(hipMemcpy(c->d_dirty + edge, &one, sizeof(int), hipMemcpyHostToDevice));
  MV_CHECK(launch_gather_stream(c));
  MV_HIP(hipStreamSynchronize(c->stream));
  return MVICP_OK;
} MVICP_GUARD_ABI

int mvicp_nn_query(mvicp_ctx* c, int frame, const double* queries, int n, int nn_method, int* idx, double* d2) try {
  MV_CHECK(bind(c));
  if (frame < 0 || frame >= c->n_frames) { set_error("frame %d out of range", frame); return MVICP_ERR_ARG; }
  if (n < 0 || (n && (!queries || !idx || !d2))) { set_error("bad query buffers"); return MVICP_ERR_ARG; }
  MV_CHECK(finish_builds(c));
  const FrameDev& f = c->frames[frame];
  if (f.n == 0) { set_error("frame %d is empty (nanoflann throws here: nanoflann.hpp:904)", frame); return MVICP_ERR_STATE; }
  if (n == 0) return MVICP_OK;
  double* dq = nullptr; int* di = nullptr; double* dd = nullptr;
  MV_CHECK(dev_alloc(&dq, 3 * (size_t)n)); MV_CHECK(dev_alloc(&di, (size_t)n)); MV_CHECK(dev_alloc(&dd, (size_t)n));
  MV_HIP(hipMemcpy(dq, queries, sizeof(double) * 3 * (size_t)n, hipMemcpyHostToDevice));
  int method = (nn_method == MVICP_NN_AUTO || nn_method == MVICP_NN_TILE) ? MVICP_NN_GRID : nn_method;
  if (c->tie_rule) MV_CHECK(ensure_tie_trees(c, std::vector<int>(1, frame)));
  c->tie_skip = false;
  if (method == MVICP_NN_GRID && !f.has_grid) method = MVICP_NN_BRUTE;
  int st;
  if (method == MVICP_NN_BRUTE) st = launch_nn_brute_queries(c, f, dq, n, di, dd);
  else if (method == MVICP_NN_GRID) st = launch_nn_grid_queries(c, f, dq, n, di, dd);
  else { set_error("unknown nn_method %d", nn_method); st = MVICP_ERR_ARG; }
  if (st == MVICP_OK) {
    hipError_t e1 = hipStreamSynchronize(c->stream);
    if (e1 == hipSuccess) census_resolve(c);
    hipError_t e2 = hipMemcpy(idx, di, sizeof(int) * n, hipMemcpyDeviceToHost);
    hipError_t e3 = hipMemcpy(d2, dd, sizeof(double) * n, hipMemcpyDeviceToHost);
    if (e1 != hipSuccess || e2 != hipSuccess || e3 != hipSuccess) { set_error("nn_query copy-back failed"); st = MVICP_ERR_HIP; }
  }
  dev_free(dq); dev_free(di); dev_free(dd);
  if (c->profile) prof_collect_lazy(c);
  return st;
} MVICP_GUARD_ABI

int mvicp_linearize(mvicp_ctx* c, const double* poses, int point_to_plane, int robust, double* out) try {
  MV_CHECK(bind(c));
  if (!poses || !out) { set_error("null argument"); return MVICP_ERR_ARG; }
  if (c->E == 0) { set_error("no graph"); return MVICP_ERR_STATE; }
  MV_CHECK(evaluate_blocks(c, poses, point_to_plane, robust, out));
  if (c->profile) prof_collect_lazy(c);
  return MVICP_OK;
} MVICP_GUARD_ABI

int mvicp_linearize_pair(mvicp_ctx* c, const double* poses_a, const double* poses_b, int point_to_plane, int robust, double* out_a, double* out_b) try {
  MV_CHECK(bind(c));
  if (!poses_a || !poses_b || !out_a || !out_b) { set_error("null argument"); return MVICP_ERR_ARG; }
  if (c->E == 0) { set_error("no graph"); return MVICP_ERR_STATE; }
  if (c->comm || c->ar_fn) {
    MV_CHECK(evaluate_blocks(c, poses_a, point_to_plane, robust, out_a));
    MV_CHECK(evaluate_blocks(c, poses_b, point_to_plane, robust, out_b));
  } else {
    MV_CHECK(evaluate_pair(c, poses_a, poses_b, point_to_plane, robust, out_a, out_b));
  }
  if (c->profile) prof_collect_lazy(c);
  return MVICP_OK;
} MVICP_GUARD_ABI

int mvicp_set_option(mvicp_ctx* c, const char* name, double value) try {
  MV_CHECK(bind(c));
  if (!name) { set_error("null option name"); return MVICP_ERR_ARG; }
  if (std::strcmp(name, "async_build") == 0) { c->async_build = value != 0.0; return MVICP_OK; }
  if (std::strcmp(name, "grid_target") == 0 || std::strcmp(name, "grid_curve") == 0) MV_CHECK(finish_builds(c));
  if (std::strcmp(name, "nn_tree_only") == 0) { c->nn_tree_only = value != 0.0; return MVICP_OK; }
  if (std::strcmp(name, "nn_cache") == 0) { c->nn_cache_enable = value != 0.0; c->nn_cache_valid = false; return MVICP_OK; }
  if (std::strcmp(name, "lin_chunk") == 0) { c->lin_chunk_override = (int)value; return MVICP_OK; }
  if (std::strcmp(name, "list_reuse") == 0) { c->list_reuse = value != 0.0; return MVICP_OK; }
  if (std::strcmp(name, "lin_interleave") == 0) { c->lin_interleave = value != 0.0; return MVICP_OK; }
  if (std::strcmp(name, "lin_share_p") == 0) { c->lin_share_p = value != 0.0; return MVICP_OK; }
  if (std::strcmp(name, "lin_pair") == 0) { c->lin_pair = value != 0.0; return MVICP_OK; }
  if (std::strcmp(name, "nn_census") == 0) { c->nn_census = value != 0.0; return MVICP_OK; }
  if (std::strcmp(name, "nn_skip_far") == 0) { c->nn_skip_far = value != 0.0; return MVICP_OK; }
  if (std::strcmp(name, "sel_bracket") == 0) { c->sel_bracket = value != 0.0; return MVICP_OK; }
  if (std::strcmp(name, "prune_rho") == 0) { c->prune_rho = value; return MVICP_OK; }
  if (std::strcmp(name, "grid_curve") == 0) { c->grid_curve = (int)value; return MVICP_OK; }
  if (std::strcmp(name, "auto_settle") == 0) { c->auto_settle = value; return MVICP_OK; }
  if (std::strcmp(name, "auto_switch") == 0) { c->auto_switch = value; return MVICP_OK; }
  if (std::strcmp(name, "nn_cell") == 0) { c->nn_cell = value != 0.0; return MVICP_OK; }
  if (std::strcmp(name, "nn_search_factor") == 0) { if (!(value >= 0.0)) { set_error("nn_search_factor < 0"); return MVICP_ERR_ARG; } c->nn_search_factor = value; c->nn_cache_valid = false; return MVICP_OK; }
  if (std::strcmp(name, "tie_rule") == 0) { c->tie_rule = value != 0.0; return MVICP_OK; }
  if (std::strcmp(name, "tie_lazy") == 0) { c->tie_lazy = value != 0.0; return MVICP_OK; }
  if (std::strcmp(name, "tile_seed") == 0) { c->tile_seed = value != 0.0; return MVICP_OK; }
  if (std::strcmp(name, "tile_bounds") == 0) { c->tile_bounds = (int)value; return MVICP_OK; }
  if (std::strcmp(name, "tile_mu") == 0) { if (!(value > 0.0 && value <= 1.0)) { set_error("tile_mu outside (0, 1]"); return MVICP_ERR_ARG; } c->tile_mu = value; return MVICP_OK; }
  if (std::strcmp(name, "mfma_kacc") == 0) { if (!(value >= 1.0 && value <= 1024.0)) { set_error("mfma_kacc outside [1, 1024]"); return MVICP_ERR_ARG; } c->mfma_kacc = value; return MVICP_OK; }
  if (std::strcmp(name, "mfma_lbt") == 0) { c->mfma_lbt = (int)value; return MVICP_OK; }
  if (std::strcmp(name, "mfma_entry") == 0) { c->mfma_entry = (int)value; return MVICP_OK; }
  if (std::strcmp(name, "mfma_trig") == 0) { c->mfma_trig = (int)value; return MVICP_OK; }
  if (std::strcmp(name, "tile_mfma") == 0) { c->tile_mfma = (int)value; return MVICP_OK; }
  if (std::strcmp(name, "tile_waves") == 0) { c->tile_waves = (int)value; return MVICP_OK; }
  if (std::strcmp(name, "cache_mfma_ratio") == 0) { c->cache_mfma_ratio = value; return MVICP_OK; }
  if (std::strcmp(name, "reject_cache") == 0) { c->reject_cache = value != 0.0; return MVICP_OK; }
  if (std::strcmp(name, "tile_miss") == 0) { if (!(value >= 0.0 && value <= 64.0)) { set_error("tile_miss outside [0, 64]"); return MVICP_ERR_ARG; } c->tile_miss = (int)value; return MVICP_OK; }
  if (std::strcmp(name, "tile_cache") == 0) { c->tile_cache = (int)value; return MVICP_OK; }
  if (std::strcmp(name, "spin_wait") == 0) { c->spin_wait = value != 0.0; return MVICP_OK; }
  if (std::strcmp(name, "fault_inject") == 0) { c->fault_inject = (int)value; return MVICP_OK; }
  if (std::strcmp(name, "fault_inject_build") == 0) { c->fault_inject_build.store((int)value); return MVICP_OK; }
  if (std::strcmp(name, "fault_inject_eval") == 0) { c->fault_inject_eval = (int)value; return MVICP_OK; }
  if (std::strcmp(name, "spec_eval") == 0) { c->spec_enable = value != 0.0; c->spec_ready = false; c->spec2_ready = false; return MVICP_OK; }
  if (std::strcmp(name, "spec2_eval") == 0) { c->spec2_enable = value != 0.0; c->spec2_ready = false; return MVICP_OK; }
  if (std::strcmp(name, "grid_target") == 0) {
    if (!(value >= 0.5 && value <= 64.0)) { set_error("grid_target out of range"); return MVICP_ERR_ARG; }
    c->grid_target = value;
    return MVICP_OK;
  }
  set_error("unknown option '%s'", name);
  return MVICP_ERR_ARG;
} MVICP_GUARD_ABI
int mvicp_nn_census_ex(mvicp_ctx* c, double* out, int cap) try {
  MV_CHECK(bind(c));
  if (!out || cap < 0) { set_error("bad output buffer"); return MVICP_ERR_ARG; }
  const double v[10] = {c->nn_queries, c->nn_candidates, c->nn_nodes, c->nn_far, c->nn_hits, c->nn_fetched, c->nn_dbg[0], c->nn_dbg[1], c->nn_dbg[2], c->nn_dbg[3]};
  const int n = std::min(cap, 10);
  for (int i = 0; i < n; ++i) out[i] = v[i];
  return n;
} MVICP_GUARD_ABI
int mvicp_nn_census(mvicp_ctx* c, double* out5) try {
  const int n = mvicp_nn_census_ex(c, out5, 5);
  return n < 0 ? n : MVICP_OK;
} MVICP_GUARD_ABI

int mvicp_profile_enable(mvicp_ctx* c, int on) try {
  MV_CHECK(bind(c));
  c->profile = on != 0;
  c->profile_level = on;
  return MVICP_OK;
} MVICP_GUARD_ABI
int mvicp_profile_reset(mvicp_ctx* c) try {
  MV_CHECK(bind(c));
  MV_HIP(hipStreamSynchronize(c->stream));
  prof_collect(c);
  for (auto& kv : c->prof) { kv.second.ms = 0; kv.second.launches = 0; kv.second.bytes = 0; kv.second.survey_bytes = 0; kv.second.queries = 0; }
  c->nn_candidates = c->nn_nodes = c->nn_far = c->nn_queries = c->nn_hits = c->nn_fetched = 0;
  for (int k = 0; k < 4; ++k) c->nn_dbg[k] = 0;
  return MVICP_OK;
} MVICP_GUARD_ABI
static void prof_sum(mvicp_ctx* c, const char* kernel, double out[5]) {
  for (int k = 0; k < 5; ++k) out[k] = 0.0;
  const std::string key = kernel ? kernel : "";
  for (const auto& kv : c->prof) {
    if (!(kv.first == key || (key == "nn" && kv.first.compare(0, 3, "nn_") == 0))) continue;
    out[0] += kv.second.ms;
    if (key == "nn" && (kv.first == "nn_far" || kv.first == "nn_tie")) continue;
    out[1] += (double)kv.second.launches; out[2] += kv.second.bytes; out[3] += kv.second.survey_bytes; out[4] += kv.second.queries;
  }
}
int mvicp_profile_get(mvicp_ctx* c, const char* kernel, double* total_ms, long long* launches, double* alg_bytes) try {
  MV_CHECK(bind(c));
  MV_HIP(hipStreamSynchronize(c->stream));
  prof_collect(c);
  double v[5];
  prof_sum(c, kernel, v);
  if (total_ms) *total_ms = v[0];
  if (launches) *launches = (long long)v[1];
  if (alg_bytes) *alg_bytes = v[2];
  return MVICP_OK;
} MVICP_GUARD_ABI
int mvicp_profile_get_ex(mvicp_ctx* c, const char* kernel, double* out, int cap) try {
  MV_CHECK(bind(c));
  if (!out || cap < 0) { set_error("bad output buffer"); return MVICP_ERR_ARG; }
  MV_HIP(hipStreamSynchronize(c->stream));
  prof_collect(c);
  double v[5];
  prof_sum(c, kernel, v);
  const int n = std::min(cap, 5);
  for (int k = 0; k < n; ++k) out[k] = v[k];
  return n;
} MVICP_GUARD_ABI
void* mvicp_stream(mvicp_ctx* c) { return c ? (void*)c->stream : nullptr; }
int mvicp_sync(mvicp_ctx* c) try {
  MV_CHECK(bind(c));
  MV_HIP(hipStreamSynchronize(c->stream));
  return MVICP_OK;
} MVICP_GUARD_ABI

}
```

mv-lm-icp_amd/csrc/common.h:

```cpp
#pragma once
#include <hip/hip_runtime.h>

#include <atomic>
#include <cstdarg>
#include <cstdio>
#include <future>
#include <map>
#include <memory>
#include <string>
#include <vector>

#include "../../include/mvicp.h"
#include "abi_guard.h"

namespace mvicp {

void set_error(const char* fmt, ...);

#define MV_HIP(expr)                                                                          \
  do {                                                                                        \
    hipError_t _e = (expr);                                                                   \
    if (_e != hipSuccess) {                                                                   \
      mvicp::set_error("%s:%d: %s -> %s", __FILE__, __LINE__, #expr, hipGetErrorString(_e));  \
      return MVICP_ERR_HIP;                                                                   \
    }                                                                                         \
  } while (0)

#define MV_CHECK(call)            \
  do {                            \
    int _s = (call);              \
    if (_s != MVICP_OK) return _s; \
  } while (0)

constexpr int kLinPartial = 32;
constexpr int kLinThreads = 256;
constexpr int kCompactBlock = 1024;
constexpr int kSelBlock = 8192;
constexpr int kEdgeXf = 40;
constexpr int kEdgeRel = 12;

struct GridDev {
  int dims[3] = {0, 0, 0};
  double origin[3] = {0, 0, 0};
  double cell = 0.0, inv_cell = 0.0;
  int n_cells = 0;
  double* spts = nullptr;
  int* sidx = nullptr;
  void* srec = nullptr;
  void* crec = nullptr;
  double* snor = nullptr;
  int* inv = nullptr;
  std::vector<int> h_order, h_inv;
  void* table = nullptr;
  unsigned int table_mask = 0; int table_shift = 0;
  float* oct = nullptr;
  int oct_leaf = 0; long long oct_first_leaf = 0;
  float* wide = nullptr;
  double maxabs = 0.0;
  int wide_levels = 0;
  int wide_cnt[6] = {0, 0, 0, 0, 0, 0};
  long long wide_off[6] = {0, 0, 0, 0, 0, 0};
  void* mf_ops = nullptr; void* mf_blk = nullptr;
  double struct_bytes = 0.0;
  void* bricks = nullptr; void* celltab = nullptr; int bdims[3] = {0, 0, 0};
  size_t celltab_bytes = 0;
  int* ov_samp = nullptr; int ov_samp_s = 0;
};

struct PointRec { double x, y, z; long long idx; };

struct BuildJob { std::future<int> fut; std::string err; std::vector<double> xyz, nrm; };

struct DevBounds { double lo[3], hi[3], max_norm, maxabs, wall_ms; int nonfinite, pad; };

struct FrameDev {
  std::shared_ptr<BuildJob> job;
  std::string build_error;
  int n = 0;
  double* pts = nullptr;
  double* nor = nullptr;
  GridDev grid;
  bool has_grid = false;
  double max_norm = 0.0;
  double build_ms[2] = {0.0, -1.0};
  void* tie_nodes = nullptr; int* tie_ord = nullptr; int* tie_slot = nullptr; double tie_box[6] = {0, 0, 0, 0, 0, 0}; bool has_tie = false;
};

struct ProfEntry {
  double ms = 0.0;
  long long launches = 0;
  double bytes = 0.0;
  double survey_bytes = 0.0;
  double queries = 0.0;
  std::vector<std::pair<hipEvent_t, hipEvent_t>> pending;
  std::vector<hipEvent_t> pool;
};

struct RcclApi;

}

struct mvicp_ctx {
  int device = 0;
  hipStream_t stream = nullptr;
  int n_frames = 0;
  std::vector<mvicp::FrameDev> frames;

  int rank = 0, world = 1;
  int E = 0;
  std::vector<int> esrc, edst;
  std::vector<char> owned;
  std::vector<long long> cap_off;
  long long total_cap = 0;
  std::vector<int> h_count;
  std::vector<float> h_weight;
  bool have_corr = false;

  double* d_ctl = nullptr; size_t ctl_r1 = 0, ctl_rel2_off = 0, ctl_r2_off = 0, ctl_r2 = 0;
  int* d_esrc = nullptr; int* d_edst = nullptr;
  long long* d_cap_off = nullptr;
  int* d_nsrc = nullptr;
  int* d_count = nullptr;
  double* d_a = nullptr;
  double* d_xf = nullptr;
  double* d_rel = nullptr;
  double* d_rel2 = nullptr;
  int* d_nn_idx = nullptr; double* d_nn_d2 = nullptr;
  float* d_nn_lb = nullptr;
  bool nn_cache_valid = false; bool nn_cache_enable = true; float nn_cache_thresh = -1.f;
  std::vector<char> nn_cache_edge;
  std::vector<double> prev_q;
  std::vector<double> prev_xf;
  int* d_first = nullptr; int* d_second = nullptr; double* d_cd2 = nullptr;
  int* d_qpos = nullptr;
  int* d_dirty = nullptr;
  int* d_dirty_slots = nullptr; int* d_dslot_off = nullptr; std::vector<int> dslot_off; int n_dslots = 0;
  std::vector<char> list_valid;
  std::vector<char> explicit_list;
  void* d_export = nullptr; void* h_export = nullptr; size_t export_cap = 0;
  int* d_xblock_cnt = nullptr;
  std::vector<long long> export_off;
  bool export_valid = false;
  std::vector<hipEvent_t> export_events; std::vector<int> export_edge_chunk; int export_chunks = 0; bool export_in_flight = false;
  std::vector<char> qpos_valid;
  std::vector<unsigned long long> corr_epoch;
  unsigned long long epoch_counter = 0;
  double* d_stream = nullptr;
  int n_cblocks = 0;
  std::vector<int> cblock_off;
  int* d_cblock_off = nullptr; int* d_cblock_cnt = nullptr;
  void* d_sel_state = nullptr; unsigned int* d_sel_hist = nullptr; double* d_median = nullptr;
  int n_sblocks = 0; std::vector<int> sblock_off; int* d_sblock_off = nullptr;
  double* d_sel_lohi = nullptr;
  std::vector<double> sel_med1, sel_med2;
  bool sel_bracket = true;
  bool bracket_counters_clean = false;
  double* d_sel_keys1 = nullptr; double* d_sel_keys2 = nullptr;
  bool lin_interleave = true;
  bool lin_share_p = true;
  int lin_chunk_override = 0;
  int lin_chunk = 4096;
  int n_chunks = 0;
  std::vector<int> chunk_first;
  int* d_chunk_edge = nullptr; int* d_chunk_start = nullptr; int* d_chunk_first = nullptr;
  double* d_partials = nullptr;
  bool lin_pair = true;
  double* d_out = nullptr;
  double* d_res_target = nullptr;
  double* h_pin = nullptr; size_t h_pin_doubles = 0;
  size_t pin_blocks_off = 0, pin_res_off = 0, pin_misc_off = 0;
  double* d_res_host = nullptr;
  double* d_blocks_host = nullptr;
  double* lin_out = nullptr;
  bool spec_enable = true; bool spec_flags_valid = false; int spec_param = 0, spec_plane = 0, spec_robust = 0;
  int spec_q_plane = 0, spec_q_robust = 0;
  bool spec_arm = false;
  bool spec_ready = false;
  std::vector<double> spec_poses;
  size_t pin_spec_off = 0, pin_adev_off = 0; double* d_spec_host = nullptr; double* d_adev_host = nullptr;
  bool spec2_enable = true, spec2_armed = false, spec2_ready = false; int spec2_plane = 0, spec2_robust = 0;
  std::vector<double> spec2_poses;
  std::vector<double> last_cand_poses;
  int last_cand_plane = -1, last_cand_robust = -1;
  size_t pin_spec2_off = 0, pin_rel2_off = 0; double* d_spec2_host = nullptr;
  size_t pin_blocks2_off = 0; double* d_blocks2_host = nullptr;
  double* d_a_check = nullptr;
  bool spin_wait = false;
  unsigned long long* h_census = nullptr;
  bool census_pending = false; double census_nq = 0; int census_kind = 0; const char* census_scope = "nn_grid";
  int* d_split_idx = nullptr; double* d_split_d2 = nullptr; size_t split_cap = 0;

  char* ov_dev = nullptr; char* ov_pin = nullptr; size_t ov_bytes = 0;

  struct CachedTable { std::vector<char> bytes; void* d = nullptr; size_t cap = 0; };
  std::map<std::string, CachedTable> tables;
  char* d_scratch = nullptr; size_t scratch_bytes = 0, scratch_used = 0;
  std::vector<char> active;

  mvicp::RcclApi* rccl = nullptr;
  void* comm = nullptr;
  mvicp_allreduce_fn ar_fn = nullptr; void* ar_user = nullptr;
  std::vector<double> ar_host;

  bool async_build = true;
  std::atomic<int> fault_inject_build{0};
  int fault_inject = 0, fault_inject_eval = 0;
  bool list_reuse = true;
  bool nn_tree_only = false;
  bool nn_census = false;
  void* d_census = nullptr; size_t census_bytes = 0;
  void* d_far_list = nullptr; size_t far_cap = 0; unsigned int* d_far_count = nullptr;
  int far_parity = 0;
  unsigned int* h_far_seen = nullptr; unsigned int* d_far_seen = nullptr;
  bool prev_grid_kernel = false;
  bool far_skip = false;
  bool far_narrow = false;
  bool skip_dirty_reduce = false;
  bool nn_skip_far = false;
  double nn_search_factor = 4.0;
  bool tie_lazy = true;
  bool tie_rule = true;
  unsigned long long* d_tie_list = nullptr; size_t tie_cap = 0; unsigned int* d_tie_count = nullptr; int tie_parity = 0;
  unsigned int* h_tie_seen = nullptr; unsigned int* d_tie_seen = nullptr;
  unsigned int corr_tie_seen = 1u, corr_far_seen = 1u;
  bool tie_skip = false;
  bool tile_seed = true;
  int tile_bounds = 1;
  int tile_cache = 1;
  double cache_mfma_ratio = 3.0;
  bool cached_on_mfma = false;
  bool reject_cache = true;
  int tile_miss = 8;
  double tile_mu = 0.02;
  int tile_mfma = 1;
  double mfma_kacc = 34.0;
  int mfma_lbt = 1;
  int mfma_entry = 0;
  int mfma_trig = 2;
  int tile_waves = 0;
  double auto_prev_dist = 0.0; int auto_last_method = -1; double auto_settle = 0.5;
  double last_rms = -1.0;
  bool nn_cell = false;
  double auto_switch = 1.0;
  double prune_rho = 0.05;
  int grid_curve = 2;
  double grid_target = 5.0;
  double nn_candidates = 0, nn_nodes = 0, nn_far = 0, nn_queries = 0, nn_hits = 0, nn_fetched = 0;
  double nn_dbg[4] = {0, 0, 0, 0};

  bool profile = false; int profile_level = 0;
  std::map<std::string, mvicp::ProfEntry> prof;
};

namespace mvicp {

int launch_nn_brute_edges(mvicp_ctx* c);
int launch_nn_brute_queries(mvicp_ctx* c, const FrameDev& f, const double* d_q, int n, int* d_idx, double* d_d2);
int launch_nn_grid_edges(mvicp_ctx* c, double d2_bound);
double search_bound(const mvicp_ctx* c, double d2_bound);
int launch_nn_tile_edges(mvicp_ctx* c, double d2_bound, bool with_bounds, bool with_cache, bool with_list);
int launch_nn_mfma_edges(mvicp_ctx* c, double d2_bound, bool with_bounds, bool with_cache, bool with_list);
int build_mfma(FrameDev& f, const double* sorted_pts);
int warm_nn_mfma(mvicp_ctx* c);
int warm_nn_tile(mvicp_ctx* c); int warm_nn_grid(mvicp_ctx* c);
int build_wide(FrameDev& f, const double* sorted_pts);
int launch_nn_grid_queries(mvicp_ctx* c, const FrameDev& f, const double* d_q, int n, int* d_idx, double* d_d2);
int build_grid(mvicp_ctx* c, FrameDev& f, const double* h_xyz);
int device_bounds(hipStream_t stream, const double* d_xyz, int n, DevBounds* out);
int build_grid_device(mvicp_ctx* c, FrameDev& f, const DevBounds& b, int grid_curve, double grid_target);
int finish_builds(mvicp_ctx* c);
void free_grid(GridDev& g);
void free_tie(FrameDev& f);
int overlap_census(mvicp_ctx* c, const double* xf, double B2, double scale, int max_samples, int* samples, int* hits, long long* sumq);
void free_overlap(mvicp_ctx* c);
int launch_compact(mvicp_ctx* c, double d2_bound);
int launch_gather_stream(mvicp_ctx* c);
int launch_select_median(mvicp_ctx* c);
int launch_export(mvicp_ctx* c);
int launch_select_bracket(mvicp_ctx* c);
int launch_linearize(mvicp_ctx* c, int plane, int robust);
int launch_linearize_pair(mvicp_ctx* c, int plane, int robust, double* out_a, double* out_b);
int launch_normals(mvicp_ctx* c, FrameDev& f, int k, int* d_knn);
int stream_wait(mvicp_ctx* c);
void census_resolve(mvicp_ctx* c);

int cached_upload(mvicp_ctx* c, const char* key, const void* src, size_t bytes, void** dptr);
void scratch_reset(mvicp_ctx* c);
int scratch_upload(mvicp_ctx* c, const void* src, size_t bytes, void** dptr);

struct ProfScope {
  mvicp_ctx* c; const char* name; hipEvent_t a = nullptr, b = nullptr; bool on;
  ProfScope(mvicp_ctx* c, const char* name, double bytes);
  ~ProfScope();
};
void prof_collect(mvicp_ctx* c);
void prof_collect_lazy(mvicp_ctx* c);
struct HostScope {
  mvicp_ctx* c; const char* name; double t0; bool on;
  HostScope(mvicp_ctx* c, const char* name);
  ~HostScope();
};

}
```

mv-lm-icp_amd/csrc/corr.hip:

```cpp
#include "common.h"

namespace mvicp {

namespace {

constexpr int NT = 256;
constexpr int IPT = kCompactBlock / NT;

__device__ __forceinline__ int find_edge(const int* __restrict__ off, int E, int b) {
  int lo = 0, hi = E;
  while (hi - lo > 1) {
    const int mid = (lo + hi) >> 1;
    if (off[mid] <= b) lo = mid; else hi = mid;
  }
  return lo;
}

__device__ __forceinline__ int block_exclusive_scan(int v, int* __restrict__ wave_tot, int* total) {
  const int lane = threadIdx.x & 63, wave = threadIdx.x >> 6;
  int inc = v;
#pragma unroll
  for (int d = 1; d < 64; d <<= 1) {
    const int o = __shfl_up(inc, d, 64);
    if (lane >= d) inc += o;
  }
  if (lane == 63) wave_tot[wave] = inc;
  __syncthreads();
  int base = 0, tot = 0;
#pragma unroll
  for (int w = 0; w < NT / 64; ++w) {
    const int t = wave_tot[w];
    if (w < wave) base += t;
    tot += t;
  }
  *total = tot;
  return base + inc - v;
}

__global__ __launch_bounds__(NT) void count_kernel(const int* __restrict__ cblock_off, int E, const int* __restrict__ nsrc,
                                                   const long long* __restrict__ cap_off, const int* __restrict__ nn_idx,
                                                   const double* __restrict__ nn_d2, double bound, int* __restrict__ cblock_cnt,
                                                   const int* __restrict__ dirty) {
  __shared__ int wave_tot[NT / 64];
  const int b = blockIdx.x;
  const int e = find_edge(cblock_off, E, b);
  if (dirty[e] == 0) return;
  const int lb = b - cblock_off[e];
  const int n = nsrc[e];
  const long long base = cap_off[e];
  int cnt = 0;
#pragma unroll
  for (int i = 0; i < IPT; ++i) {
    const int k = lb * kCompactBlock + threadIdx.x * IPT + i;
    if (k < n) cnt += (nn_idx[base + k] >= 0 && nn_d2[base + k] < bound) ? 1 : 0;
  }
  int total;
  block_exclusive_scan(cnt, wave_tot, &total);
  if (threadIdx.x == 0) cblock_cnt[b] = total;
}

__global__ __launch_bounds__(NT) void scan_kernel(const int* __restrict__ cblock_off, int* __restrict__ cblock_cnt, int* __restrict__ count,
                                                  const int* __restrict__ dirty) {
  __shared__ int wave_tot[NT / 64];
  __shared__ int carry_s;
  const int e = blockIdx.x;
  if (dirty[e] == 0) return;
  const int b0 = cblock_off[e], b1 = cblock_off[e + 1];
  if (threadIdx.x == 0) carry_s = 0;
  __syncthreads();
  for (int s = b0; s < b1; s += NT) {
    const int b = s + threadIdx.x;
    const int v = (b < b1) ? cblock_cnt[b] : 0;
    int total;
    const int ex = block_exclusive_scan(v, wave_tot, &total);
    const int carry = carry_s;
    if (b < b1) cblock_cnt[b] = carry + ex;
    __syncthreads();
    if (threadIdx.x == 0) carry_s = carry + total;
    __syncthreads();
  }
  if (threadIdx.x == 0) count[e] = carry_s;
}

__global__ __launch_bounds__(NT) void scatter_kernel(const int* __restrict__ cblock_off, int E, const int* __restrict__ nsrc,
                                                     const long long* __restrict__ cap_off, const int* __restrict__ nn_idx,
                                                     const double* __restrict__ nn_d2, double bound, const int* __restrict__ cblock_cnt,
                                                     int* __restrict__ first, int* __restrict__ second, double* __restrict__ cd2,
                                                     int* __restrict__ qpos, const int* __restrict__ dirty) {
  __shared__ int wave_tot[NT / 64];
  const int b = blockIdx.x;
  const int e = find_edge(cblock_off, E, b);
  if (dirty[e] == 0) return;
  const int lb = b - cblock_off[e];
  const int n = nsrc[e];
  const long long base = cap_off[e];
  int idx[IPT];
  double d2[IPT];
  bool ok[IPT];
  int cnt = 0;
#pragma unroll
  for (int i = 0; i < IPT; ++i) {
    const int k = lb * kCompactBlock + threadIdx.x * IPT + i;
    ok[i] = false;
    if (k < n) {
      idx[i] = nn_idx[base + k];
      d2[i] = nn_d2[base + k];
      ok[i] = idx[i] >= 0 && d2[i] < bound;
    }
    cnt += ok[i] ? 1 : 0;
  }
  int total;
  int pos = cblock_cnt[b] + block_exclusive_scan(cnt, wave_tot, &total);
#pragma unroll
  for (int i = 0; i < IPT; ++i) {
    const int k = lb * kCompactBlock + threadIdx.x * IPT + i;
    if (k < n) qpos[base + k] = ok[i] ? pos : -1;
    if (!ok[i]) continue;
    first[base + pos] = k;
    second[base + pos] = idx[i];
    cd2[base + pos] = d2[i];
    ++pos;
  }
}

__global__ __launch_bounds__(NT) void gather_kernel(const int* __restrict__ cblock_off, int E, const int* __restrict__ count,
                                                    const long long* __restrict__ cap_off, long long total_cap, const int* __restrict__ first,
                                                    const int* __restrict__ second, const PointRec* const* __restrict__ src_rec,
                                                    const PointRec* const* __restrict__ dst_rec, const double* const* __restrict__ dst_nor,
                                                    double* __restrict__ stream, const int* __restrict__ dirty) {
  const int b = blockIdx.x;
  const int e = find_edge(cblock_off, E, b);
  if (dirty[e] == 0) return;
  const int lb = b - cblock_off[e];
  const int cnt = count[e];
  if (lb * kCompactBlock >= cnt) return;
  const long long base = cap_off[e];
  const PointRec* __restrict__ sp = src_rec[e];
  const PointRec* __restrict__ dp = dst_rec[e];
  const double* __restrict__ dn = dst_nor[e];
  for (int i = 0; i < IPT; ++i) {
    const int pos = lb * kCompactBlock + i * NT + threadIdx.x;
    if (pos >= cnt) break;
    const size_t f = (size_t)first[base + pos], s = (size_t)second[base + pos];
    const size_t o = (size_t)(base + pos);
    const double2* pa = reinterpret_cast<const double2*>(sp + f);
    const double2 a0 = pa[0], a1 = pa[1];
    const double2* pb = reinterpret_cast<const double2*>(dp + s);
    const double2 b0 = pb[0], b1 = pb[1];
    __builtin_nontemporal_store(a0.x, &stream[0 * total_cap + o]);
    __builtin_nontemporal_store(a0.y, &stream[1 * total_cap + o]);
    __builtin_nontemporal_store(a1.x, &stream[2 * total_cap + o]);
    __builtin_nontemporal_store(b0.x, &stream[7 * total_cap + o]);
    __builtin_nontemporal_store(b0.y, &stream[8 * total_cap + o]);
    __builtin_nontemporal_store(b1.x, &stream[9 * total_cap + o]);
    if (dn != nullptr) {
      const double n0 = dn[3 * s], n1 = dn[3 * s + 1], n2 = dn[3 * s + 2];
      __builtin_nontemporal_store(n0, &stream[3 * total_cap + o]);
      __builtin_nontemporal_store(n1, &stream[4 * total_cap + o]);
      __builtin_nontemporal_store(n2, &stream[5 * total_cap + o]);
      __builtin_nontemporal_store(n0 * b0.x + n1 * b0.y + n2 * b1.x, &stream[6 * total_cap + o]);
    }
  }
}

constexpr int kSelBins = 2048;
struct SelState { unsigned long long prefix; int k; int pad; };

template <int PER, typename F>
__device__ __forceinline__ void pick_bin(F get, unsigned int k, int* __restrict__ wave_tot, int* __restrict__ sh_pick, int& bin, unsigned int& below) {
  unsigned int h[PER];
  int mine = 0;
#pragma unroll
  for (int i = 0; i < PER; ++i) { h[i] = get(threadIdx.x * PER + i); mine += (int)h[i]; }
  int total;
  const int ex = block_exclusive_scan(mine, wave_tot, &total);
  if (threadIdx.x == 0) { sh_pick[0] = NT * PER - 1; sh_pick[1] = total; }
  __syncthreads();
  if ((unsigned int)ex <= k && k < (unsigned int)(ex + mine)) {
    unsigned int cum = (unsigned int)ex;
#pragma unroll
    for (int i = 0; i < PER; ++i) {
      if (cum + h[i] > k) { sh_pick[0] = threadIdx.x * PER + i; sh_pick[1] = (int)cum; break; }
      cum += h[i];
    }
  }
  __syncthreads();
  bin = sh_pick[0]; below = (unsigned int)sh_pick[1];
  __syncthreads();
}

template <int PASS>
__global__ __launch_bounds__(NT) void select_pass_kernel(const int* __restrict__ sblock_off, int E, const int* __restrict__ count,
                                                         const long long* __restrict__ cap_off, const double* __restrict__ in_keys,
                                                         const unsigned int* __restrict__ in_cnt, unsigned int* __restrict__ hist,
                                                         const SelState* __restrict__ state,
                                                         double* __restrict__ out_keys, unsigned int* __restrict__ out_cnt) {
  constexpr int SPT = kSelBlock / NT;
  constexpr int SHIFT = PASS == 0 ? 52 : PASS == 1 ? 41 : 30;
  __shared__ unsigned int lh[kSelBins];
  __shared__ int wave_tot[NT / 64];
  __shared__ unsigned int sh_base;
  const int b = blockIdx.x;
  const int e = find_edge(sblock_off, E, b);
  const int lb = b - sblock_off[e];
  const int cnt = count[e];
  const int n_in = PASS == 2 ? (cnt > 0 ? (int)in_cnt[e] : 0) : cnt;
  if ((long long)lb * kSelBlock >= n_in) return;
  SelState st;
  st.prefix = 0ull; st.k = cnt / 2; st.pad = 0;
  if (PASS > 0) st = state[(size_t)(PASS - 1) * E + e];
  for (int i = threadIdx.x; i < kSelBins; i += NT) lh[i] = 0u;
  __syncthreads();
  const long long base = cap_off[e];
  unsigned long long keys[SPT];
  int nmatch = 0;
#pragma unroll
  for (int i = 0; i < SPT; ++i) {
    const int pos = lb * kSelBlock + i * NT + threadIdx.x;
    bool match = pos < n_in;
    unsigned long long key = 0ull;
    if (match) {
      key = (unsigned long long)__double_as_longlong(__builtin_nontemporal_load(&in_keys[base + pos]));
      if (PASS > 0) match = (key >> (SHIFT + 11)) == (st.prefix >> (SHIFT + 11));
    }
    const unsigned int bin = (unsigned int)(key >> SHIFT) & (kSelBins - 1);
    if (PASS == 0) {
      const int lane = threadIdx.x & 63;
      const bool inwin = match && bin >= 768u && bin < 1024u;
      if (inwin) atomicAdd(&lh[(bin & 255u) | ((unsigned int)(lane & 7) << 8)], 1u);
      unsigned long long todo = __ballot(match && !inwin);
      while (todo) {
        const int leader = __ffsll((long long)todo) - 1;
        const unsigned int lbin = (unsigned int)__builtin_amdgcn_readlane((int)bin, leader);
        const unsigned long long same = __ballot(match && !inwin && bin == lbin) & todo;
        if (lane == leader) atomicAdd(&hist[((size_t)PASS * E + e) * kSelBins + lbin], (unsigned int)__popcll(same));
        todo &= ~same;
      }
    } else if (match) {
      atomicAdd(&lh[bin], 1u);
    }
    keys[i] = key;
    if (PASS > 0 && match) { keys[i] |= 1ull << 63; ++nmatch; }
  }
  if (PASS > 0) {
    int total;
    int off = block_exclusive_scan(nmatch, wave_tot, &total);
    if (threadIdx.x == 0) sh_base = total ? atomicAdd(&out_cnt[e], (unsigned int)total) : 0u;
    __syncthreads();
    off += (int)sh_base;
#pragma unroll
    for (int i = 0; i < SPT; ++i)
      if (keys[i] >> 63) out_keys[base + off++] = __longlong_as_double((long long)(keys[i] & ~(1ull << 63)));
  }
  __syncthreads();
  if (PASS == 0) {
    unsigned int v = 0;
#pragma unroll
    for (int cpy = 0; cpy < 8; ++cpy) v += lh[cpy * 256 + threadIdx.x];
    if (v) atomicAdd(&hist[((size_t)PASS * E + e) * kSelBins + 768 + threadIdx.x], v);
  } else {
    for (int i = threadIdx.x; i < kSelBins; i += NT) {
      const unsigned int v = lh[i];
      if (v) atomicAdd(&hist[((size_t)PASS * E + e) * kSelBins + i], v);
    }
  }
}

template <int PASS>
__global__ __launch_bounds__(NT) void select_pick_kernel(int E, const int* __restrict__ count, const unsigned int* __restrict__ hist,
                                                         SelState* __restrict__ state) {
  constexpr int SHIFT = PASS == 0 ? 52 : 41;
  __shared__ int wave_tot[NT / 64];
  __shared__ int sh_pick[2];
  const int e = blockIdx.x;
  const int cnt = count[e];
  if (cnt <= 0) return;
  SelState st;
  st.prefix = 0ull; st.k = cnt / 2; st.pad = 0;
  if (PASS > 0) st = state[(size_t)(PASS - 1) * E + e];
  const unsigned int* hp = hist + ((size_t)PASS * E + e) * kSelBins;
  int bin; unsigned int below;
  pick_bin<kSelBins / NT>([&](int i) { return hp[i]; }, (unsigned int)st.k, wave_tot, sh_pick, bin, below);
  if (threadIdx.x == 0) {
    SelState o;
    o.prefix = st.prefix | ((unsigned long long)bin << SHIFT);
    o.k = st.k - (int)below; o.pad = 0;
    state[(size_t)PASS * E + e] = o;
  }
}

__device__ __forceinline__ void write_a_scale(int cnt, double med, int e, double* __restrict__ a_dev, double* __restrict__ a_host) {
  if (a_dev == nullptr) return;
  const double a = cnt > 0 ? (double)(float)__dmul_rn(sqrt(med), 1.5) : 0.0;
  a_dev[e] = a;
  if (a_host) a_host[e] = a;
}

__global__ __launch_bounds__(NT) void select_final_kernel(int E, const int* __restrict__ count, const long long* __restrict__ cap_off,
                                                          const double* __restrict__ keys2, const unsigned int* __restrict__ cnt2,
                                                          const unsigned int* __restrict__ hist, const SelState* __restrict__ state,
                                                          double* __restrict__ median, double* __restrict__ host_res,
                                                          double* __restrict__ a_dev, double* __restrict__ a_host, double armed) {
  __shared__ unsigned int lh[1024];
  __shared__ int wave_tot[NT / 64];
  __shared__ int sh_pick[2];
  const int e = blockIdx.x;
  const int cnt = count[e];
  double med = 0.0;
  if (cnt > 0) {
    SelState st = state[(size_t)1 * E + e];
    {
      const unsigned int* hp = hist + ((size_t)2 * E + e) * kSelBins;
      int bin; unsigned int below;
      pick_bin<kSelBins / NT>([&](int i) { return hp[i]; }, (unsigned int)st.k, wave_tot, sh_pick, bin, below);
      st.prefix |= (unsigned long long)bin << 30;
      st.k -= (int)below;
    }
    const int n2 = (int)cnt2[e];
    const long long base = cap_off[e];
    for (int shift = 20; shift >= 0; shift -= 10) {
      for (int i = threadIdx.x; i < 1024; i += NT) lh[i] = 0u;
      __syncthreads();
      for (int pos = threadIdx.x; pos < n2; pos += NT) {
        const unsigned long long key = (unsigned long long)__double_as_longlong(keys2[base + pos]);
        if ((key >> (shift + 10)) == (st.prefix >> (shift + 10))) atomicAdd(&lh[(key >> shift) & 1023ull], 1u);
      }
      __syncthreads();
      int bin; unsigned int below;
      pick_bin<1024 / NT>([&](int i) { return lh[i]; }, (unsigned int)st.k, wave_tot, sh_pick, bin, below);
      st.prefix |= (unsigned long long)bin << shift;
      st.k -= (int)below;
    }
    med = __longlong_as_double((long long)st.prefix);
  }
  if (threadIdx.x == 0) {
    median[e] = med;
    if (host_res) {
      host_res[2 * e] = (double)(cnt > 0 ? cnt : 0); host_res[2 * e + 1] = med;
      if (e == 0) host_res[2 * E] = armed;
    }
    write_a_scale(cnt, med, e, a_dev, a_host);
  }
}

__global__ __launch_bounds__(NT) void bracket_pass_kernel(const int* __restrict__ sblock_off, int E, const int* __restrict__ count,
                                                          const long long* __restrict__ cap_off, const double* __restrict__ keys,
                                                          const double* __restrict__ lohi, unsigned int* __restrict__ cnt_lt,
                                                          double* __restrict__ out_keys, unsigned int* __restrict__ out_cnt) {
  constexpr int SPT = kSelBlock / NT;
  __shared__ unsigned int s_lt[NT / 64];
  __shared__ unsigned int s_mid, s_base;
  const int b = blockIdx.x;
  const int e = find_edge(sblock_off, E, b);
  const int lb = b - sblock_off[e];
  const int cnt = count[e];
  if ((long long)lb * kSelBlock >= cnt) return;
  if (threadIdx.x == 0) s_mid = 0u;
  __syncthreads();
  const unsigned long long lo = (unsigned long long)__double_as_longlong(lohi[2 * e]), hi = (unsigned long long)__double_as_longlong(lohi[2 * e + 1]);
  const long long base = cap_off[e];
  const int lane = threadIdx.x & 63, wave = threadIdx.x >> 6;
  unsigned int nlt = 0, nmid = 0;
  unsigned long long kept[SPT];
#pragma unroll
  for (int i = 0; i < SPT / 2; ++i) {
    const int pos = lb * kSelBlock + 2 * (i * NT + threadIdx.x);
    unsigned long long k0 = ~0ull, k1 = ~0ull;
    if (pos + 1 < cnt) {
      typedef double d2v __attribute__((ext_vector_type(2)));
      const d2v v = __builtin_nontemporal_load(reinterpret_cast<const d2v*>(keys + base + pos));
      k0 = (unsigned long long)__double_as_longlong(v.x); k1 = (unsigned long long)__double_as_longlong(v.y);
    } else if (pos < cnt) {
      k0 = (unsigned long long)__double_as_longlong(keys[base + pos]);
    }
    nlt += (k0 < lo ? 1u : 0u) + (k1 < lo ? 1u : 0u);
    const bool m0 = k0 >= lo && k0 <= hi, m1 = k1 >= lo && k1 <= hi;
    kept[2 * i] = m0 ? k0 : ~0ull; kept[2 * i + 1] = m1 ? k1 : ~0ull;
    nmid += (m0 ? 1u : 0u) + (m1 ? 1u : 0u);
  }
  unsigned int off = nmid ? atomicAdd(&s_mid, nmid) : 0u;
  unsigned int w = nlt;
#pragma unroll
  for (int d = 32; d >= 1; d >>= 1) w += __shfl_xor(w, d, 64);
  if (lane == 0) s_lt[wave] = w;
  __syncthreads();
  if (threadIdx.x == 0) {
    const unsigned int t = s_lt[0] + s_lt[1] + s_lt[2] + s_lt[3];
    if (t) atomicAdd(&cnt_lt[e], t);
    s_base = s_mid ? atomicAdd(&out_cnt[e], s_mid) : 0u;
  }
  __syncthreads();
  if (nmid) {
    off += s_base;
#pragma unroll
    for (int i = 0; i < SPT; ++i)
      if (kept[i] != ~0ull) out_keys[base + off++] = __longlong_as_double((long long)kept[i]);
  }
}

__global__ __launch_bounds__(NT) void bracket_final_kernel(int E, const int* __restrict__ count, const long long* __restrict__ cap_off,
                                                           const double* __restrict__ keys1, unsigned int* __restrict__ cnt_lt,
                                                           unsigned int* __restrict__ cnt_mid, double* __restrict__ median,
                                                           double* __restrict__ host_res, double* __restrict__ a_dev, double* __restrict__ a_host, double armed) {
  __shared__ unsigned int lh[kSelBins];
  __shared__ int wave_tot[NT / 64];
  __shared__ int sh_pick[2];
  const int e = blockIdx.x;
  const int cnt = count[e];
  double med = 0.0;
  bool ok = true;
  if (cnt > 0) {
    const unsigned int k = (unsigned int)(cnt / 2), nlt = cnt_lt[e], nmid = cnt_mid[e];
    ok = nlt <= k && k < nlt + nmid;
    if (ok) {
      unsigned long long prefix = 0ull;
      unsigned int rank = k - nlt;
      const long long base = cap_off[e];
      constexpr int KR = 8;
      const bool in_regs = nmid <= (unsigned int)(KR * NT);
      unsigned long long kreg[KR];
#pragma unroll
      for (int i = 0; i < KR; ++i) {
        const unsigned int pos = threadIdx.x + i * NT;
        kreg[i] = (in_regs && pos < nmid) ? (unsigned long long)__double_as_longlong(keys1[base + pos]) : ~0ull;
      }
      int hi_bit = 63;
#pragma unroll 1
      for (int pass = 0; pass < 6; ++pass) {
        const int bits = pass < 3 ? 11 : 10;
        const int shift = hi_bit - bits;
        for (int i = threadIdx.x; i < kSelBins; i += NT) lh[i] = 0u;
        __syncthreads();
        if (in_regs) {
#pragma unroll
          for (int i = 0; i < KR; ++i) {
            const unsigned long long key = kreg[i];
            if ((key >> hi_bit) == (prefix >> hi_bit)) atomicAdd(&lh[(key >> shift) & ((1ull << bits) - 1ull)], 1u);
          }
        } else {
          for (unsigned int pos = threadIdx.x; pos < nmid; pos += NT) {
            const unsigned long long key = (unsigned long long)__double_as_longlong(keys1[base + pos]);
            if ((key >> hi_bit) == (prefix >> hi_bit)) atomicAdd(&lh[(key >> shift) & ((1ull << bits) - 1ull)], 1u);
          }
        }
        __syncthreads();
        int bin; unsigned int below;
        pick_bin<kSelBins / NT>([&](int i) { return lh[i]; }, rank, wave_tot, sh_pick, bin, below);
        prefix |= (unsigned long long)bin << shift;
        rank -= below;
        hi_bit = shift;
      }
      med = __longlong_as_double((long long)prefix);
    }
  }
  if (threadIdx.x == 0) {
    if (ok) median[e] = med;
    host_res[2 * e] = (double)(cnt > 0 ? cnt : 0);
    host_res[2 * e + 1] = ok ? med : -1.0;
    if (e == 0) host_res[2 * E] = armed;
    write_a_scale(ok ? cnt : 0, med, e, a_dev, a_host);
  }
  __syncthreads();
  if (threadIdx.x == 0) { cnt_lt[e] = 0u; cnt_mid[e] = 0u; }
}

}

int launch_compact(mvicp_ctx* c, double d2_bound) {
  if (c->n_cblocks == 0) return MVICP_OK;
  double bytes = 0;
  for (int e = 0; e < c->E; ++e) if (c->owned[e]) bytes += 2.0 * 12.0 * c->frames[c->esrc[e]].n;
  ProfScope ps(c, "compact", bytes);
  hipLaunchKernelGGL(count_kernel, dim3(c->n_cblocks), dim3(NT), 0, c->stream, c->d_cblock_off, c->E, c->d_nsrc, c->d_cap_off, c->d_nn_idx,
                     c->d_nn_d2, d2_bound, c->d_cblock_cnt, c->d_dirty);
  hipLaunchKernelGGL(scan_kernel, dim3(c->E), dim3(NT), 0, c->stream, c->d_cblock_off, c->d_cblock_cnt, c->d_count, c->d_dirty);
  hipLaunchKernelGGL(scatter_kernel, dim3(c->n_cblocks), dim3(NT), 0, c->stream, c->d_cblock_off, c->E, c->d_nsrc, c->d_cap_off, c->d_nn_idx,
                     c->d_nn_d2, d2_bound, c->d_cblock_cnt, c->d_first, c->d_second, c->d_cd2, c->d_qpos, c->d_dirty);
  MV_HIP(hipGetLastError());
  return MVICP_OK;
}

int launch_gather_stream(mvicp_ctx* c) {
  if (c->n_cblocks == 0) return MVICP_OK;
  std::vector<const void*> tab(3 * (size_t)c->E, nullptr);
  for (int e = 0; e < c->E; ++e) {
    tab[e] = c->frames[c->esrc[e]].grid.srec;
    tab[c->E + e] = c->frames[c->edst[e]].grid.srec;
    tab[2 * c->E + e] = c->frames[c->edst[e]].grid.snor;
  }
  const void** d_tab = nullptr;
  MV_CHECK(cached_upload(c, "gather_tab", tab.data(), sizeof(void*) * tab.size(), (void**)&d_tab));
  {
    ProfScope ps(c, "gather", 0.0);
    hipLaunchKernelGGL(gather_kernel, dim3(c->n_cblocks), dim3(NT), 0, c->stream, c->d_cblock_off, c->E, c->d_count, c->d_cap_off, c->total_cap,
                       c->d_first, c->d_second, (const PointRec* const*)d_tab, (const PointRec* const*)(d_tab + c->E), (const double* const*)(d_tab + 2 * c->E), c->d_stream, c->d_dirty);
  }
  MV_HIP(hipGetLastError());
  return MVICP_OK;
}

int launch_select_bracket(mvicp_ctx* c) {
  if (c->E == 0) return MVICP_OK;
  double bytes = 0;
  for (int e = 0; e < c->E; ++e) if (c->owned[e]) bytes += 8.0 * c->h_count[e];
  ProfScope ps(c, "select", bytes);
  const size_t E = (size_t)c->E;
  unsigned int* cnt_lt = c->d_sel_hist;
  unsigned int* cnt_mid = cnt_lt + E;
  if (c->n_sblocks) {
    if (!c->bracket_counters_clean) MV_HIP(hipMemsetAsync(cnt_lt, 0, sizeof(unsigned int) * 2 * E, c->stream));
    c->bracket_counters_clean = true;
    hipLaunchKernelGGL(bracket_pass_kernel, dim3(c->n_sblocks), dim3(NT), 0, c->stream, c->d_sblock_off, c->E, c->d_count, c->d_cap_off, c->d_cd2,
                       (const double*)c->d_sel_lohi, cnt_lt, c->d_sel_keys1, cnt_mid);
  }
  hipLaunchKernelGGL(bracket_final_kernel, dim3(c->E), dim3(NT), 0, c->stream, c->E, c->d_count, c->d_cap_off, c->d_sel_keys1, cnt_lt,
                     cnt_mid, c->d_median, c->d_res_target ? c->d_res_target : c->d_res_host, c->spec_arm ? c->d_a : (double*)nullptr,
                     c->spec_arm ? c->d_a_check : (double*)nullptr, c->spec_arm ? 1.0 : 0.0);
  MV_HIP(hipGetLastError());
  return MVICP_OK;
}

int launch_select_median(mvicp_ctx* c) {
  if (c->E == 0) return MVICP_OK;
  double bytes = 0;
  for (int e = 0; e < c->E; ++e) if (c->owned[e]) bytes += 16.0 * c->h_count[e];
  ProfScope ps(c, "select", bytes);
  const size_t E = (size_t)c->E;
  unsigned int* hist = c->d_sel_hist;
  unsigned int* cnt1 = hist + 3 * E * kSelBins;
  unsigned int* cnt2 = cnt1 + E;
  SelState* st = (SelState*)c->d_sel_state;
  c->bracket_counters_clean = false;
  if (c->n_sblocks) {
    MV_HIP(hipMemsetAsync(hist, 0, sizeof(unsigned int) * (3 * E * kSelBins + 2 * E), c->stream));
    const dim3 grid(c->n_sblocks), blk(NT);
    hipLaunchKernelGGL((select_pass_kernel<0>), grid, blk, 0, c->stream, c->d_sblock_off, c->E, c->d_count, c->d_cap_off, c->d_cd2, (const unsigned int*)nullptr,
                       hist, (const SelState*)st, (double*)nullptr, (unsigned int*)nullptr);
    hipLaunchKernelGGL((select_pick_kernel<0>), dim3(c->E), blk, 0, c->stream, c->E, c->d_count, (const unsigned int*)hist, st);
    hipLaunchKernelGGL((select_pass_kernel<1>), grid, blk, 0, c->stream, c->d_sblock_off, c->E, c->d_count, c->d_cap_off, c->d_cd2, (const unsigned int*)nullptr,
                       hist, (const SelState*)st, c->d_sel_keys1, cnt1);
    hipLaunchKernelGGL((select_pick_kernel<1>), dim3(c->E), blk, 0, c->stream, c->E, c->d_count, (const unsigned int*)hist, st);
    hipLaunchKernelGGL((select_pass_kernel<2>), grid, blk, 0, c->stream, c->d_sblock_off, c->E, c->d_count, c->d_cap_off, c->d_sel_keys1, (const unsigned int*)cnt1,
                       hist, (const SelState*)st, c->d_sel_keys2, cnt2);
  }
  hipLaunchKernelGGL(select_final_kernel, dim3(c->E), dim3(NT), 0, c->stream, c->E, c->d_count, c->d_cap_off, c->d_sel_keys2, (const unsigned int*)cnt2,
                     (const unsigned int*)hist, (const SelState*)st, c->d_median, c->d_res_target ? c->d_res_target : c->d_res_host,
                     c->spec_arm ? c->d_a : (double*)nullptr, c->spec_arm ? c->d_a_check : (double*)nullptr, c->spec_arm ? 1.0 : 0.0);
  MV_HIP(hipGetLastError());
  return MVICP_OK;
}

}
```

Measured before the change: 1120 iterations/s.

## Replace three-pass radix median select with bound-anchored histogram plus bracket pass

Rewrites the median selection fallback: instead of three radix histogram passes plus a final refinement kernel, it builds one histogram of exponent-aligned bins anchored at the d2 bound, picks a lo/hi bracket, and reuses the existing bracket pass/final kernels. The pick kernel re-zeroes the histogram and scratch is tracked as clean, removing the per-call memset. It also adds a sel_reuse path that skips selection entirely when nothing can change and a prior result is still valid. The costs are extra state flags that must be invalidated correctly, and a bracket that may be wide if many keys fall in one bin.

```diff
diff --git a/mv-lm-icp_amd/csrc/api.cpp b/mv-lm-icp_amd/csrc/api.cpp
--- a/mv-lm-icp_amd/csrc/api.cpp
+++ b/mv-lm-icp_amd/csrc/api.cpp
@@ -142,9 +142,9 @@
   dev_free(c->d_esrc); dev_free(c->d_edst); dev_free(c->d_cap_off); dev_free(c->d_count);
   dev_free(c->d_ctl); c->d_nsrc = nullptr; c->d_a = nullptr; c->d_xf = nullptr; c->d_rel = nullptr; c->d_rel2 = nullptr; c->d_dirty = nullptr;
   dev_free(c->d_nn_idx); dev_free(c->d_nn_d2); dev_free(c->d_nn_lb); dev_free(c->d_first); dev_free(c->d_second);
-  dev_free(c->d_sblock_off); dev_free(c->d_sel_keys1); dev_free(c->d_sel_keys2); c->n_sblocks = 0;
-  dev_free(c->d_cd2); dev_free(c->d_qpos); dev_free(c->d_dirty_slots); dev_free(c->d_dslot_off); dev_free(c->d_stream); dev_free(c->d_cblock_off); dev_free(c->d_cblock_cnt); if (c->d_sel_state) (void)hipFree(c->d_sel_state);
-  c->d_sel_state = nullptr; dev_free(c->d_sel_hist); dev_free(c->d_median); dev_free(c->d_chunk_edge); dev_free(c->d_chunk_start);
+  dev_free(c->d_sblock_off); dev_free(c->d_sel_keys1); c->n_sblocks = 0;
+  dev_free(c->d_cd2); dev_free(c->d_qpos); dev_free(c->d_dirty_slots); dev_free(c->d_dslot_off); dev_free(c->d_stream); dev_free(c->d_cblock_off); dev_free(c->d_cblock_cnt);
+  dev_free(c->d_sel_hist); dev_free(c->d_median); dev_free(c->d_chunk_edge); dev_free(c->d_chunk_start);
   dev_free(c->d_chunk_first); dev_free(c->d_partials); dev_free(c->d_out);
   if (c->h_pin) (void)hipHostFree(c->h_pin);
   c->h_pin = nullptr; c->h_pin_doubles = 0; c->d_res_host = nullptr; c->d_blocks_host = nullptr; c->lin_out = nullptr;
@@ -865,13 +865,15 @@
   MV_HIP(hipMemset(c->d_dirty_slots, 0, sizeof(int) * std::max<size_t>((size_t)c->n_dslots, 1)));
   MV_HIP(hipMemcpy(c->d_dslot_off, c->dslot_off.data(), sizeof(int) * (E + 1), hipMemcpyHostToDevice));
   MV_CHECK(dev_alloc(&c->d_cblock_off, E + 1)); MV_CHECK(dev_alloc(&c->d_cblock_cnt, (size_t)c->n_cblocks));
-  MV_HIP(hipMalloc(&c->d_sel_state, 16 * 3 * (size_t)std::max(E, 1))); MV_CHECK(dev_alloc(&c->d_sel_hist, (size_t)E * (3 * 2048 + 5)));
+  MV_CHECK(dev_alloc(&c->d_sel_hist, (size_t)E * (2048 + 2)));
+  MV_HIP(hipMemset(c->d_sel_hist, 0, sizeof(unsigned int) * std::max<size_t>((size_t)E * (2048 + 2), 1)));
+  c->sel_scratch_clean = true; c->sel_result_valid = false; c->sel_result_armed = false;
   c->sblock_off.assign(E + 1, 0);
   for (int e = 0; e < E; ++e) c->sblock_off[e + 1] = c->sblock_off[e] + (int)(((c->owned[e] ? c->frames[src[e]].n : 0) + kSelBlock - 1) / kSelBlock);
   c->n_sblocks = c->sblock_off[E];
   MV_CHECK(dev_alloc(&c->d_sblock_off, (size_t)E + 1));
   MV_HIP(hipMemcpy(c->d_sblock_off, c->sblock_off.data(), sizeof(int) * (E + 1), hipMemcpyHostToDevice));
-  MV_CHECK(dev_alloc(&c->d_sel_keys1, cap)); MV_CHECK(dev_alloc(&c->d_sel_keys2, cap));
+  MV_CHECK(dev_alloc(&c->d_sel_keys1, cap));
   if (cap > c->far_cap) {
     if (c->d_far_list) MV_HIP(hipFree(c->d_far_list));
     c->d_far_list = nullptr; c->far_cap = 0;
@@ -922,7 +924,7 @@
     c->d_spec2_host = (double*)dp + c->pin_spec2_off;
     c->d_blocks2_host = (double*)dp + c->pin_blocks2_off;
   }
-  c->spec_ready = false; c->spec_arm = false; c->bracket_counters_clean = false;
+  c->spec_ready = false; c->spec_arm = false;
   c->spec2_ready = false; c->spec2_armed = false; c->last_cand_poses.clear();
   c->prev_xf.assign((size_t)E * 24, 0.0);
   if (!c->h_census) MV_HIP(hipHostMalloc((void**)&c->h_census, 8 * sizeof(unsigned long long), hipHostMallocDefault));
@@ -941,6 +943,7 @@
   c->qpos_valid.assign(E, 0);
   for (int e = 0; e < E; ++e) c->corr_epoch[e] = ++c->epoch_counter;
   c->sel_med1.assign(E, -1.0); c->sel_med2.assign(E, -1.0);
+  c->sel_result_valid = false;
   c->spec_ready = false; c->spec_arm = false; c->spec_flags_valid = false;
   c->spec2_ready = false; c->spec2_armed = false; c->last_cand_poses.clear();
   c->have_corr = false;
@@ -972,7 +975,16 @@
   return MVICP_OK;
 } MVICP_GUARD_ABI
 
+static int correspond_body(mvicp_ctx* c, const double* poses, const unsigned char* fixed, float thresh, int nn_method, int* counts, float* weights, bool* tie_unresolved);
+
 static int correspond_once(mvicp_ctx* c, const double* poses, const unsigned char* fixed, float thresh, int nn_method, int* counts, float* weights, bool* tie_unresolved) {
+  struct Guard { mvicp_ctx* c; bool ok = false; ~Guard() { if (!ok) { c->sel_result_valid = false; c->sel_scratch_clean = false; } } } guard{c};
+  const int st = correspond_body(c, poses, fixed, thresh, nn_method, counts, weights, tie_unresolved);
+  guard.ok = st == MVICP_OK;
+  return st;
+}
+
+static int correspond_body(mvicp_ctx* c, const double* poses, const unsigned char* fixed, float thresh, int nn_method, int* counts, float* weights, bool* tie_unresolved) {
   if (!poses) { set_error("poses is null"); return MVICP_ERR_ARG; }
   if (c->E == 0) { set_error("no graph: call mvicp_set_graph first"); return MVICP_ERR_STATE; }
   const int E = c->E;
@@ -1116,6 +1128,7 @@
                  c->last_cand_plane == c->spec_q_plane && c->last_cand_robust == c->spec_q_robust;
     if (spec2_plan && c->lin_pair) fill_rel_into(c, c->last_cand_poses.data(), hx + c->ctl_rel2_off);
   }
+  const bool sel_skip = !exchange && c->sel_reuse && nothing_can_change && c->sel_result_valid && (!c->spec_arm || c->sel_result_armed);
   if (method != MVICP_NN_BRUTE && method != MVICP_NN_GRID && method != MVICP_NN_TILE) { set_error("unknown nn_method %d", nn_method); return MVICP_ERR_ARG; }
   bool all_unchanged = true;
   for (int e = 0; e < E; ++e) { if (!unchanged[e]) all_unchanged = false; if (c->active[e]) c->qpos_valid[e] = 0; }
@@ -1150,7 +1163,8 @@
     MV_CHECK(launch_compact(c, bound));
     MV_CHECK(launch_gather_stream(c));
   }
-  return use_bracket ? launch_select_bracket(c) : launch_select_median(c);
+  if (sel_skip) { c->h_pin[c->pin_res_off + 2 * (size_t)E] = c->spec_arm ? 1.0 : 0.0; return MVICP_OK; }
+  return use_bracket ? launch_select_bracket(c) : launch_select_median(c, bound);
   };
   if (st_local == MVICP_OK) st_local = local_search();
   if (st_local != MVICP_OK && !exchange) { c->spec_flags_valid = false; return st_local; }
@@ -1217,7 +1231,7 @@
     for (int e = 0; e < E; ++e) if (hr[2 * e + 1] < 0.0) redo = true;
     if (redo) {
       spec_bad = true;
-      int st_r = launch_select_median(c);
+      int st_r = launch_select_median(c, bound);
       if (exchange) {
         int st_x = MVICP_OK;
         if (st_r != MVICP_OK) {
@@ -1262,6 +1276,8 @@
   c->spec_ready = c->spec_arm && !spec_bad;
   c->spec2_ready = c->spec_ready && c->spec2_armed;
   c->spec2_armed = false;
+  if (!sel_skip) c->sel_result_armed = c->spec_arm;
+  c->sel_result_valid = !exchange;
   c->spec_arm = false;
   double* ha = c->h_pin + c->ctl_r2_off + (size_t)E * kEdgeRel;
   for (int e = 0; e < E; ++e) {
@@ -1398,6 +1414,7 @@
   c->list_valid[edge] = 0; c->explicit_list[edge] = 1; c->export_valid = false;
   c->qpos_valid[edge] = 0; c->corr_epoch[edge] = ++c->epoch_counter;
   c->sel_med1[edge] = c->sel_med2[edge] = -1.0;
+  c->sel_result_valid = false;
   const double a = (double)weight;
   MV_HIP(hipMemcpy(c->d_count + edge, &n, sizeof(int), hipMemcpyHostToDevice));
   {
@@ -1485,6 +1502,7 @@
   if (std::strcmp(name, "nn_census") == 0) { c->nn_census = value != 0.0; return MVICP_OK; }
   if (std::strcmp(name, "nn_skip_far") == 0) { c->nn_skip_far = value != 0.0; return MVICP_OK; }
   if (std::strcmp(name, "sel_bracket") == 0) { c->sel_bracket = value != 0.0; return MVICP_OK; }
+  if (std::strcmp(name, "sel_reuse") == 0) { c->sel_reuse = value != 0.0; return MVICP_OK; }
   if (std::strcmp(name, "prune_rho") == 0) { c->prune_rho = value; return MVICP_OK; }
   if (std::strcmp(name, "grid_curve") == 0) { c->grid_curve = (int)value; return MVICP_OK; }
   if (std::strcmp(name, "auto_settle") == 0) { c->auto_settle = value; return MVICP_OK; }
diff --git a/mv-lm-icp_amd/csrc/common.h b/mv-lm-icp_amd/csrc/common.h
--- a/mv-lm-icp_amd/csrc/common.h
+++ b/mv-lm-icp_amd/csrc/common.h
@@ -149,13 +149,17 @@
   int n_cblocks = 0;
   std::vector<int> cblock_off;
   int* d_cblock_off = nullptr; int* d_cblock_cnt = nullptr;
-  void* d_sel_state = nullptr; unsigned int* d_sel_hist = nullptr; double* d_median = nullptr;
+  unsigned int* d_sel_hist = nullptr;
+  double* d_median = nullptr;
   int n_sblocks = 0; std::vector<int> sblock_off; int* d_sblock_off = nullptr;
   double* d_sel_lohi = nullptr;
   std::vector<double> sel_med1, sel_med2;
   bool sel_bracket = true;
-  bool bracket_counters_clean = false;
-  double* d_sel_keys1 = nullptr; double* d_sel_keys2 = nullptr;
+  bool sel_scratch_clean = false;
+  bool sel_reuse = true;
+  bool sel_result_valid = false;
+  bool sel_result_armed = false;
+  double* d_sel_keys1 = nullptr;
   bool lin_interleave = true;
   bool lin_share_p = true;
   int lin_chunk_override = 0;
@@ -275,7 +279,7 @@
 void free_overlap(mvicp_ctx* c);
 int launch_compact(mvicp_ctx* c, double d2_bound);
 int launch_gather_stream(mvicp_ctx* c);
-int launch_select_median(mvicp_ctx* c);
+int launch_select_median(mvicp_ctx* c, double d2_bound);
 int launch_export(mvicp_ctx* c);
 int launch_select_bracket(mvicp_ctx* c);
 int launch_linearize(mvicp_ctx* c, int plane, int robust);
diff --git a/mv-lm-icp_amd/csrc/corr.hip b/mv-lm-icp_amd/csrc/corr.hip
--- a/mv-lm-icp_amd/csrc/corr.hip
+++ b/mv-lm-icp_amd/csrc/corr.hip
@@ -1,4 +1,6 @@
 #include "common.h"
+
+#include <cstring>
 
 namespace mvicp {
 
@@ -164,7 +166,12 @@
 }
 
 constexpr int kSelBins = 2048;
-struct SelState { unsigned long long prefix; int k; int pad; };
+constexpr int kSelShift = 46;
+
+__device__ __forceinline__ unsigned int sel_bin(unsigned long long key, long long kbq) {
+  const long long d = kbq - (long long)(key >> kSelShift);
+  return d <= 0 ? (unsigned int)(kSelBins - 1) : d >= kSelBins - 1 ? 0u : (unsigned int)(kSelBins - 1 - d);
+}
 
 template <int PER, typename F>
 __device__ __forceinline__ void pick_bin(F get, unsigned int k, int* __restrict__ wave_tot, int* __restrict__ sh_pick, int& bin, unsigned int& below) {
@@ -189,103 +196,61 @@
   __syncthreads();
 }
 
-template <int PASS>
-__global__ __launch_bounds__(NT) void select_pass_kernel(const int* __restrict__ sblock_off, int E, const int* __restrict__ count,
-                                                         const long long* __restrict__ cap_off, const double* __restrict__ in_keys,
-                                                         const unsigned int* __restrict__ in_cnt, unsigned int* __restrict__ hist,
-                                                         const SelState* __restrict__ state,
-                                                         double* __restrict__ out_keys, unsigned int* __restrict__ out_cnt) {
+__global__ __launch_bounds__(NT) void select_hist_kernel(const int* __restrict__ sblock_off, int E, const int* __restrict__ count,
+                                                         const long long* __restrict__ cap_off, const double* __restrict__ keys,
+                                                         long long kbq, unsigned int* __restrict__ hist) {
   constexpr int SPT = kSelBlock / NT;
-  constexpr int SHIFT = PASS == 0 ? 52 : PASS == 1 ? 41 : 30;
   __shared__ unsigned int lh[kSelBins];
-  __shared__ int wave_tot[NT / 64];
-  __shared__ unsigned int sh_base;
   const int b = blockIdx.x;
   const int e = find_edge(sblock_off, E, b);
   const int lb = b - sblock_off[e];
   const int cnt = count[e];
-  const int n_in = PASS == 2 ? (cnt > 0 ? (int)in_cnt[e] : 0) : cnt;
-  if ((long long)lb * kSelBlock >= n_in) return;
-  SelState st;
-  st.prefix = 0ull; st.k = cnt / 2; st.pad = 0;
-  if (PASS > 0) st = state[(size_t)(PASS - 1) * E + e];
+  if ((long long)lb * kSelBlock >= cnt) return;
   for (int i = threadIdx.x; i < kSelBins; i += NT) lh[i] = 0u;
   __syncthreads();
   const long long base = cap_off[e];
-  unsigned long long keys[SPT];
-  int nmatch = 0;
-#pragma unroll
-  for (int i = 0; i < SPT; ++i) {
-    const int pos = lb * kSelBlock + i * NT + threadIdx.x;
-    bool match = pos < n_in;
-    unsigned long long key = 0ull;
-    if (match) {
-      key = (unsigned long long)__double_as_longlong(__builtin_nontemporal_load(&in_keys[base + pos]));
-      if (PASS > 0) match = (key >> (SHIFT + 11)) == (st.prefix >> (SHIFT + 11));
-    }
-    const unsigned int bin = (unsigned int)(key >> SHIFT) & (kSelBins - 1);
-    if (PASS == 0) {
-      const int lane = threadIdx.x & 63;
-      const bool inwin = match && bin >= 768u && bin < 1024u;
-      if (inwin) atomicAdd(&lh[(bin & 255u) | ((unsigned int)(lane & 7) << 8)], 1u);
-      unsigned long long todo = __ballot(match && !inwin);
-      while (todo) {
-        const int leader = __ffsll((long long)todo) - 1;
-        const unsigned int lbin = (unsigned int)__builtin_amdgcn_readlane((int)bin, leader);
-        const unsigned long long same = __ballot(match && !inwin && bin == lbin) & todo;
-        if (lane == leader) atomicAdd(&hist[((size_t)PASS * E + e) * kSelBins + lbin], (unsigned int)__popcll(same));
-        todo &= ~same;
-      }
-    } else if (match) {
-      atomicAdd(&lh[bin], 1u);
-    }
-    keys[i] = key;
-    if (PASS > 0 && match) { keys[i] |= 1ull << 63; ++nmatch; }
-  }
-  if (PASS > 0) {
-    int total;
-    int off = block_exclusive_scan(nmatch, wave_tot, &total);
-    if (threadIdx.x == 0) sh_base = total ? atomicAdd(&out_cnt[e], (unsigned int)total) : 0u;
-    __syncthreads();
-    off += (int)sh_base;
-#pragma unroll
-    for (int i = 0; i < SPT; ++i)
-      if (keys[i] >> 63) out_keys[base + off++] = __longlong_as_double((long long)(keys[i] & ~(1ull << 63)));
-  }
-  __syncthreads();
-  if (PASS == 0) {
-    unsigned int v = 0;
-#pragma unroll
-    for (int cpy = 0; cpy < 8; ++cpy) v += lh[cpy * 256 + threadIdx.x];
-    if (v) atomicAdd(&hist[((size_t)PASS * E + e) * kSelBins + 768 + threadIdx.x], v);
-  } else {
-    for (int i = threadIdx.x; i < kSelBins; i += NT) {
-      const unsigned int v = lh[i];
-      if (v) atomicAdd(&hist[((size_t)PASS * E + e) * kSelBins + i], v);
-    }
-  }
-}
-
-template <int PASS>
-__global__ __launch_bounds__(NT) void select_pick_kernel(int E, const int* __restrict__ count, const unsigned int* __restrict__ hist,
-                                                         SelState* __restrict__ state) {
-  constexpr int SHIFT = PASS == 0 ? 52 : 41;
+#pragma unroll
+  for (int i = 0; i < SPT / 2; ++i) {
+    const int pos = lb * kSelBlock + 2 * (i * NT + threadIdx.x);
+    if (pos + 1 < cnt) {
+      typedef double d2v __attribute__((ext_vector_type(2)));
+      const d2v v = __builtin_nontemporal_load(reinterpret_cast<const d2v*>(keys + base + pos));
+      atomicAdd(&lh[sel_bin((unsigned long long)__double_as_longlong(v.x), kbq)], 1u);
+      atomicAdd(&lh[sel_bin((unsigned long long)__double_as_longlong(v.y), kbq)], 1u);
+    } else if (pos < cnt) {
+      atomicAdd(&lh[sel_bin((unsigned long long)__double_as_longlong(keys[base + pos]), kbq)], 1u);
+    }
+  }
+  __syncthreads();
+  for (int i = threadIdx.x; i < kSelBins; i += NT) {
+    const unsigned int v = lh[i];
+    if (v) atomicAdd(&hist[(size_t)e * kSelBins + i], v);
+  }
+}
+
+__global__ __launch_bounds__(NT) void select_pick_kernel(int E, const int* __restrict__ count, unsigned int* __restrict__ hist, long long kbq,
+                                                         double* __restrict__ lohi) {
   __shared__ int wave_tot[NT / 64];
   __shared__ int sh_pick[2];
   const int e = blockIdx.x;
   const int cnt = count[e];
-  if (cnt <= 0) return;
-  SelState st;
-  st.prefix = 0ull; st.k = cnt / 2; st.pad = 0;
-  if (PASS > 0) st = state[(size_t)(PASS - 1) * E + e];
-  const unsigned int* hp = hist + ((size_t)PASS * E + e) * kSelBins;
+  if (cnt <= 0) {
+    if (threadIdx.x == 0) { lohi[2 * e] = 0.0; lohi[2 * e + 1] = 0.0; }
+    return;
+  }
+  unsigned int* hp = hist + (size_t)e * kSelBins;
   int bin; unsigned int below;
-  pick_bin<kSelBins / NT>([&](int i) { return hp[i]; }, (unsigned int)st.k, wave_tot, sh_pick, bin, below);
+  pick_bin<kSelBins / NT>([&](int i) { return hp[i]; }, (unsigned int)(cnt / 2), wave_tot, sh_pick, bin, below);
+#pragma unroll
+  for (int i = 0; i < kSelBins / NT; ++i) hp[threadIdx.x * (kSelBins / NT) + i] = 0u;
   if (threadIdx.x == 0) {
-    SelState o;
-    o.prefix = st.prefix | ((unsigned long long)bin << SHIFT);
-    o.k = st.k - (int)below; o.pad = 0;
-    state[(size_t)PASS * E + e] = o;
+    const long long q = kbq - (long long)(kSelBins - 1 - bin);
+    const unsigned long long low_mask = (1ull << kSelShift) - 1ull;
+    unsigned long long lo = 0ull, hi = 0ull;
+    if (bin == kSelBins - 1) { lo = (unsigned long long)(kbq > 0 ? kbq : 0) << kSelShift; hi = 0x7FFFFFFFFFFFFFFFull; }
+    else if (bin == 0) { lo = 0ull; hi = q >= 0 ? (((unsigned long long)q << kSelShift) | low_mask) : 0ull; }
+    else if (q >= 0) { lo = (unsigned long long)q << kSelShift; hi = lo | low_mask; }
+    lohi[2 * e] = __longlong_as_double((long long)lo); lohi[2 * e + 1] = __longlong_as_double((long long)hi);
   }
 }
 
@@ -294,53 +259,6 @@
   const double a = cnt > 0 ? (double)(float)__dmul_rn(sqrt(med), 1.5) : 0.0;
   a_dev[e] = a;
   if (a_host) a_host[e] = a;
-}
-
-__global__ __launch_bounds__(NT) void select_final_kernel(int E, const int* __restrict__ count, const long long* __restrict__ cap_off,
-                                                          const double* __restrict__ keys2, const unsigned int* __restrict__ cnt2,
-                                                          const unsigned int* __restrict__ hist, const SelState* __restrict__ state,
-                                                          double* __restrict__ median, double* __restrict__ host_res,
-                                                          double* __restrict__ a_dev, double* __restrict__ a_host, double armed) {
-  __shared__ unsigned int lh[1024];
-  __shared__ int wave_tot[NT / 64];
-  __shared__ int sh_pick[2];
-  const int e = blockIdx.x;
-  const int cnt = count[e];
-  double med = 0.0;
-  if (cnt > 0) {
-    SelState st = state[(size_t)1 * E + e];
-    {
-      const unsigned int* hp = hist + ((size_t)2 * E + e) * kSelBins;
-      int bin; unsigned int below;
-      pick_bin<kSelBins / NT>([&](int i) { return hp[i]; }, (unsigned int)st.k, wave_tot, sh_pick, bin, below);
-      st.prefix |= (unsigned long long)bin << 30;
-      st.k -= (int)below;
-    }
-    const int n2 = (int)cnt2[e];
-    const long long base = cap_off[e];
-    for (int shift = 20; shift >= 0; shift -= 10) {
-      for (int i = threadIdx.x; i < 1024; i += NT) lh[i] = 0u;
-      __syncthreads();
-      for (int pos = threadIdx.x; pos < n2; pos += NT) {
-        const unsigned long long key = (unsigned long long)__double_as_longlong(keys2[base + pos]);
-        if ((key >> (shift + 10)) == (st.prefix >> (shift + 10))) atomicAdd(&lh[(key >> shift) & 1023ull], 1u);
-      }
-      __syncthreads();
-      int bin; unsigned int below;
-      pick_bin<1024 / NT>([&](int i) { return lh[i]; }, (unsigned int)st.k, wave_tot, sh_pick, bin, below);
-      st.prefix |= (unsigned long long)bin << shift;
-      st.k -= (int)below;
-    }
-    med = __longlong_as_double((long long)st.prefix);
-  }
-  if (threadIdx.x == 0) {
-    median[e] = med;
-    if (host_res) {
-      host_res[2 * e] = (double)(cnt > 0 ? cnt : 0); host_res[2 * e + 1] = med;
-      if (e == 0) host_res[2 * E] = armed;
-    }
-    write_a_scale(cnt, med, e, a_dev, a_host);
-  }
 }
 
 __global__ __launch_bounds__(NT) void bracket_pass_kernel(const int* __restrict__ sblock_off, int E, const int* __restrict__ count,
@@ -499,53 +417,55 @@
   return MVICP_OK;
 }
 
+static int select_scratch(mvicp_ctx* c, unsigned int** cnt_lt, unsigned int** cnt_mid, unsigned int** hist) {
+  const size_t E = (size_t)c->E;
+  *cnt_lt = c->d_sel_hist; *cnt_mid = *cnt_lt + E; *hist = *cnt_mid + E;
+  if (!c->sel_scratch_clean) {
+    MV_HIP(hipMemsetAsync(c->d_sel_hist, 0, sizeof(unsigned int) * E * (kSelBins + 2), c->stream));
+    c->sel_scratch_clean = true;
+  }
+  return MVICP_OK;
+}
+
+static void launch_bracket_final(mvicp_ctx* c, unsigned int* cnt_lt, unsigned int* cnt_mid) {
+  hipLaunchKernelGGL(bracket_final_kernel, dim3(c->E), dim3(NT), 0, c->stream, c->E, c->d_count, c->d_cap_off, c->d_sel_keys1, cnt_lt,
+                     cnt_mid, c->d_median, c->d_res_target ? c->d_res_target : c->d_res_host, c->spec_arm ? c->d_a : (double*)nullptr,
+                     c->spec_arm ? c->d_a_check : (double*)nullptr, c->spec_arm ? 1.0 : 0.0);
+}
+
 int launch_select_bracket(mvicp_ctx* c) {
   if (c->E == 0) return MVICP_OK;
   double bytes = 0;
   for (int e = 0; e < c->E; ++e) if (c->owned[e]) bytes += 8.0 * c->h_count[e];
   ProfScope ps(c, "select", bytes);
-  const size_t E = (size_t)c->E;
-  unsigned int* cnt_lt = c->d_sel_hist;
-  unsigned int* cnt_mid = cnt_lt + E;
-  if (c->n_sblocks) {
-    if (!c->bracket_counters_clean) MV_HIP(hipMemsetAsync(cnt_lt, 0, sizeof(unsigned int) * 2 * E, c->stream));
-    c->bracket_counters_clean = true;
+  unsigned int *cnt_lt, *cnt_mid, *hist;
+  MV_CHECK(select_scratch(c, &cnt_lt, &cnt_mid, &hist));
+  if (c->n_sblocks)
     hipLaunchKernelGGL(bracket_pass_kernel, dim3(c->n_sblocks), dim3(NT), 0, c->stream, c->d_sblock_off, c->E, c->d_count, c->d_cap_off, c->d_cd2,
                        (const double*)c->d_sel_lohi, cnt_lt, c->d_sel_keys1, cnt_mid);
-  }
-  hipLaunchKernelGGL(bracket_final_kernel, dim3(c->E), dim3(NT), 0, c->stream, c->E, c->d_count, c->d_cap_off, c->d_sel_keys1, cnt_lt,
-                     cnt_mid, c->d_median, c->d_res_target ? c->d_res_target : c->d_res_host, c->spec_arm ? c->d_a : (double*)nullptr,
-                     c->spec_arm ? c->d_a_check : (double*)nullptr, c->spec_arm ? 1.0 : 0.0);
+  launch_bracket_final(c, cnt_lt, cnt_mid);
   MV_HIP(hipGetLastError());
   return MVICP_OK;
 }
 
-int launch_select_median(mvicp_ctx* c) {
+int launch_select_median(mvicp_ctx* c, double d2_bound) {
   if (c->E == 0) return MVICP_OK;
   double bytes = 0;
   for (int e = 0; e < c->E; ++e) if (c->owned[e]) bytes += 16.0 * c->h_count[e];
   ProfScope ps(c, "select", bytes);
-  const size_t E = (size_t)c->E;
-  unsigned int* hist = c->d_sel_hist;
-  unsigned int* cnt1 = hist + 3 * E * kSelBins;
-  unsigned int* cnt2 = cnt1 + E;
-  SelState* st = (SelState*)c->d_sel_state;
-  c->bracket_counters_clean = false;
+  unsigned int *cnt_lt, *cnt_mid, *hist;
+  MV_CHECK(select_scratch(c, &cnt_lt, &cnt_mid, &hist));
   if (c->n_sblocks) {
-    MV_HIP(hipMemsetAsync(hist, 0, sizeof(unsigned int) * (3 * E * kSelBins + 2 * E), c->stream));
+    long long kb;
+    std::memcpy(&kb, &d2_bound, sizeof(kb));
+    const long long kbq = kb > 0 ? kb >> kSelShift : 0;
     const dim3 grid(c->n_sblocks), blk(NT);
-    hipLaunchKernelGGL((select_pass_kernel<0>), grid, blk, 0, c->stream, c->d_sblock_off, c->E, c->d_count, c->d_cap_off, c->d_cd2, (const unsigned int*)nullptr,
-                       hist, (const SelState*)st, (double*)nullptr, (unsigned int*)nullptr);
-    hipLaunchKernelGGL((select_pick_kernel<0>), dim3(c->E), blk, 0, c->stream, c->E, c->d_count, (const unsigned int*)hist, st);
-    hipLaunchKernelGGL((select_pass_kernel<1>), grid, blk, 0, c->stream, c->d_sblock_off, c->E, c->d_count, c->d_cap_off, c->d_cd2, (const unsigned int*)nullptr,
-                       hist, (const SelState*)st, c->d_sel_keys1, cnt1);
-    hipLaunchKernelGGL((select_pick_kernel<1>), dim3(c->E), blk, 0, c->stream, c->E, c->d_count, (const unsigned int*)hist, st);
-    hipLaunchKernelGGL((select_pass_kernel<2>), grid, blk, 0, c->stream, c->d_sblock_off, c->E, c->d_count, c->d_cap_off, c->d_sel_keys1, (const unsigned int*)cnt1,
-                       hist, (const SelState*)st, c->d_sel_keys2, cnt2);
-  }
-  hipLaunchKernelGGL(select_final_kernel, dim3(c->E), dim3(NT), 0, c->stream, c->E, c->d_count, c->d_cap_off, c->d_sel_keys2, (const unsigned int*)cnt2,
-                     (const unsigned int*)hist, (const SelState*)st, c->d_median, c->d_res_target ? c->d_res_target : c->d_res_host,
-                     c->spec_arm ? c->d_a : (double*)nullptr, c->spec_arm ? c->d_a_check : (double*)nullptr, c->spec_arm ? 1.0 : 0.0);
+    hipLaunchKernelGGL(select_hist_kernel, grid, blk, 0, c->stream, c->d_sblock_off, c->E, c->d_count, c->d_cap_off, c->d_cd2, kbq, hist);
+    hipLaunchKernelGGL(select_pick_kernel, dim3(c->E), blk, 0, c->stream, c->E, c->d_count, hist, kbq, c->d_sel_lohi);
+    hipLaunchKernelGGL(bracket_pass_kernel, grid, blk, 0, c->stream, c->d_sblock_off, c->E, c->d_count, c->d_cap_off, c->d_cd2,
+                       (const double*)c->d_sel_lohi, cnt_lt, c->d_sel_keys1, cnt_mid);
+  }
+  launch_bracket_final(c, cnt_lt, cnt_mid);
   MV_HIP(hipGetLastError());
   return MVICP_OK;
 }
```

Result: faster. 1174 iterations/s (median of 6 runs) (+4.8%).
